# alex-petrenko/sample-factory

Measured on AMD Instinct MI355X. Metric: env-steps/sec (whole node), 4096 envs, 84x84x4 obs, higher is better.
Workload: dtype f32

## Files before the change

### include/sf_hip.h

```cpp
#ifndef SF_HIP_H
#define SF_HIP_H

#include <stdint.h>

#ifdef __cplusplus
extern "C" {
#endif

#define SF_OK 0
#define SF_ERR_ARG (-1)
#define SF_ERR_LAUNCH (-2)
#define SF_ERR_UNSUPPORTED (-3)

const char *sf_last_error(void);
int sf_abi_version(void);

int sf_valid_mask(const int32_t *policy_id, const float *policy_version, uint8_t *valids, uint8_t *valids_flat,
                  float *actions, int num_actions, float *log_prob_actions, int E, int T, int my_policy_id,
                  int train_step, int max_policy_lag, int32_t *num_invalid, void *stream);

int sf_gae_returns(float *rewards, const uint8_t *dones, const uint8_t *time_outs, const float *values,
                   const uint8_t *valids, const double *rms_stats, int E, int T, float gamma, float gae_lambda,
                   int value_bootstrap, float *advantages, float *returns, void *stream);

int sf_moments(const float *x, const uint8_t *valids, const int32_t *index, int64_t offset, int64_t n, int dense_x,
               double *moments, void *stream);
int sf_rms_update(const double *stats_in, const double *moments, double *stats_out, void *stream);
int sf_rms_apply(float *x, int64_t n, const double *stats, int denormalize, void *stream);

int sf_obsnorm_moments(const void *in, int in_u8, int64_t stride, const int32_t *index, int64_t offset, int traj_T,
                       int64_t n, int D, float sub_mean, float inv_scale, double *sum, double *sumsq, void *stream);
int sf_obsnorm_update(double *mean, double *var, const double *count_in, double *count_out, const double *sum,
                      const double *sumsq, int64_t n, int D, float *mu_tab, float *rstd_tab, void *stream);
int sf_obsnorm_apply(const void *in, int in_u8, int64_t stride, const int32_t *index, int64_t offset, int traj_T,
                     int64_t n, int D, int C, int HW, float sub_mean, float inv_scale, const float *mu,
                     const float *rstd, float *out, void *stream);

int sf_rnn_cell_fwd(int kind, const float *gx, const float *gh, const float *h_prev, int64_t ld_h, const float *c_prev,
                    int64_t ld_c, const float *keep, int C, int H, float *gates_out, float *h_out, float *c_out,
                    float *h_next, float *c_next, void *stream);
int sf_rnn_cell_bwd(int kind, const float *dh, const float *dc_in, const float *gates, const float *h_prev,
                    int64_t ld_h, const float *c_prev, int64_t ld_c, const float *c_out, int C, int H, float *dgx,
                    float *dgh, float *dh_direct, float *dc_prev, void *stream);
int sf_rows_add_scale(const float *a, const float *b, const float *keep, int64_t C, int H, float *y, void *stream);

int sf_vtrace(const float *params, int ld_params, const float *values, int ld_values, const float *actions,
              const float *old_logp, const float *rewards, const uint8_t *dones, const int32_t *index, int64_t offset,
              int64_t n, int A, int action_kind, int recurrence, float gamma, float rho_hat, float c_hat, float *vs,
              float *adv, const int32_t *head_n , int num_heads,
              void *stream);

typedef struct {
    float clip_ratio;
    float clip_value;
    float value_loss_coeff;
    float exploration_coeff;
    float kl_coeff;
    int32_t exploration_kind;
    int32_t action_kind;
    int32_t dense_adv;
    int32_t num_heads;
    int32_t head_n[8];
    int32_t old_values_T;
} sf_loss_cfg;

int sf_ppo_loss(const float *params, int ld_params, const float *values, int ld_values, const float *actions,
                const float *old_logp, const float *old_params, const float *old_values, const float *adv,
                const float *targets, const uint8_t *valids, const int32_t *index, int64_t offset, int64_t n, int A,
                const sf_loss_cfg *h_cfg, const double *moments, double *sums, float *g_params, float *g_values,
                float *ratio_out ,
                void *stream);
int sf_loss_scalars(const double *sums, const double *moments, const sf_loss_cfg *h_cfg, float *out, void *stream);
int sf_train_summaries(const uint8_t *valids, const float *ratio, const float *values, int ld_values,
                       const float *old_values, int old_values_T, const float *actions, int num_actions, const float *adv,
                       int dense_adv, const int32_t *policy_id, const float *policy_version, const float *action_logits,
                       int A, const int32_t *index, int64_t offset, int64_t n, int my_policy_id, int train_step,
                       float clip_ratio, const float *exp_avg_sq, int64_t P, double *out, void *stream);

int sf_minibatch_indices(int32_t *out, int64_t experience_size, int recurrence, int shuffle, uint32_t seed,
                         uint32_t epoch, void *stream);
int sf_minibatch_expand(const int32_t *chunk_starts, int32_t *out, int64_t experience_size, int recurrence,
                        void *stream);

int sf_grad_sumsq(const float *g, int64_t P, double *sumsq, void *stream);
int sf_adam_step(float *p, const float *g, float *m, float *v, int64_t P, int step, float lr, float beta1,
                 float beta2, float eps, float max_grad_norm, const double *sumsq, float grad_scale,
                 const uint32_t *skip_flag, void *stream);
int sf_adam_step_dlr(float *p, const float *g, float *m, float *v, int64_t P, int step, const float *lr_dev,
                     float lr_scale, float beta1, float beta2, float eps, float max_grad_norm, const double *sumsq,
                     float grad_scale, const uint32_t *skip_flag, void *stream);
int sf_lr_kl_adaptive(const float *kl, float *lr_dev, float threshold, float lr_min, float lr_max, float *lr_out,
                      void *stream);
int sf_clock_probe(unsigned long long *out, int spin_cycles, void *stream);

int sf_lamb_step(float *p, const float *g, float *m, float *v, float *scratch, const uint8_t *seg_id, double *seg_sums,
                 int64_t P, int num_segments, int step, float lr, float beta1, float beta2, float eps,
                 float weight_decay, float min_trust, float max_grad_norm, const double *sumsq, float grad_scale,
                 const uint32_t *skip_flag, void *stream);

int sf_sample_write_step(const float *logits, int ld_logits, const float *values, int ld_values, int B, int A, int T,
                         int t, uint32_t seed, uint32_t step, uint32_t row0, float policy_version, int deterministic,
                         int action_kind, float *traj_actions,
                         float *traj_logits, float *traj_logp, float *traj_values, float *traj_policy_version,
                         int32_t *env_actions, void *stream);

int sf_sample_write_step_masked(const float *logits, int ld_logits, const float *values, int ld_values,
                                const uint8_t *action_mask, int64_t ld_mask, int B, int A, int T, int t, uint32_t seed,
                                uint32_t step, uint32_t row0, float policy_version, int deterministic,
                                float *traj_actions, float *traj_logits, float *traj_logp, float *traj_values,
                                float *traj_policy_version, int32_t *env_actions, void *stream);

int sf_sample_write_step_tuple(const float *logits, int ld_logits, const float *values, int ld_values, int B,
                               int num_heads, const int32_t *head_n, int T, int t, uint32_t seed, uint32_t step,
                               uint32_t row0, float policy_version, int deterministic, float *traj_actions,
                               float *traj_logits, float *traj_logp, float *traj_values, float *traj_policy_version,
                               int32_t *env_actions, void *stream);

int sf_traj_write_env_step(const float *rewards, const uint8_t *terminated, const uint8_t *truncated, int B, int T,
                           int t, float reward_scale, float reward_clip, int policy_id, float *traj_rewards,
                           uint8_t *traj_dones, uint8_t *traj_time_outs, int32_t *traj_policy_id, float *ep_return,
                           int32_t *ep_len, double *ep_stats, void *stream);

int sf_synth_vec_step(float *state, const float *actions, int64_t act_stride, float *obs_out, int64_t out_stride, int B,
                      int D, int A, int env0, uint32_t seed, uint32_t step, int reset, float *rewards,
                      uint8_t *terminated, void *stream);

int sf_h2d_rows(void *dst, int64_t dst_pitch, const void *src, int64_t src_pitch, int64_t row_bytes, int64_t rows,
                void *stream);
int sf_copy_rows(void *dst, int64_t dst_pitch, const void *src, int64_t src_pitch, int64_t row_bytes, int64_t rows,
                 void *stream);

int sf_synth_obs(uint8_t *obs, int64_t env_stride, int B, int env0, int64_t obs_bytes, uint32_t seed, uint32_t step,
                 void *stream);
int sf_synth_step(const int32_t *actions, int B, int env0, int num_actions, uint32_t seed, uint32_t step,
                  float *rewards, uint8_t *terminated, void *stream);

typedef struct {
    int32_t Cin, H, W;
    int32_t Cout, KH, KW, stride;
    int32_t OH, OW;
    int32_t in_u8;
    int32_t relu;
    int32_t traj_T;
    float sub_mean, inv_scale;
} sf_conv_desc;

int64_t sf_conv_fwd_workspace(int64_t n, const sf_conv_desc *h_desc);
int sf_conv_fwd(const void *in, int64_t in_sample_stride, const int32_t *index, int64_t offset, const float *w,
                const float *bias, float *out, int64_t n, const sf_conv_desc *h_desc, void *workspace,
                int64_t workspace_bytes, void *stream);
int64_t sf_conv_wgrad_workspace(int64_t n, const sf_conv_desc *h_desc);
int sf_conv_wgrad(const void *in, int64_t in_sample_stride, const int32_t *index, int64_t offset, const float *dout,
                  float *dw, float *db, int64_t n, const sf_conv_desc *h_desc, void *workspace, void *stream);
int sf_conv_dgrad(const float *dout, const float *w, const float *in_act, float *din, int64_t n,
                  const sf_conv_desc *h_desc, void *stream);
int sf_conv_relu_mask_supported(int64_t n, const sf_conv_desc *h_desc);
int sf_conv_fwd_relu_mask(const void *in, int64_t in_sample_stride, const int32_t *index, int64_t offset, const float *w,
                          const float *bias, float *out, uint32_t *relu_mask, int64_t n, const sf_conv_desc *h_desc,
                          void *stream);
int sf_conv_wgrad_relu_mask(const void *in, int64_t in_sample_stride, const int32_t *index, int64_t offset,
                            const float *dout, const uint32_t *relu_mask, float *dw, float *db, int64_t n,
                            const sf_conv_desc *h_desc, void *workspace, void *stream);

int sf_conv_norm_supported(int64_t n, const sf_conv_desc *h_desc);
int sf_conv_fwd_norm(const void *in, int64_t in_sample_stride, const int32_t *index, int64_t offset, const float *mu,
                     const float *rstd, const float *w, const float *bias, float *out, int64_t n,
                     const sf_conv_desc *h_desc, void *stream);
int sf_conv_wgrad_norm(const void *in, int64_t in_sample_stride, const int32_t *index, int64_t offset, const float *mu,
                       const float *rstd, const float *dout, float *dw, float *db, int64_t n, const sf_conv_desc *h_desc,
                       void *workspace, void *stream);

int sf_mlp2_fwd(const float *x, int64_t x_stride, int64_t n, int D, float sub_mean, float inv_scale, const float *mu,
                const float *rstd, const float *w1, const float *b1, int H1, const float *w2, const float *b2, int H2,
                int act, float *out, void *stream);

int sf_rnn_store_state(const float *h, const float *c, const uint8_t *dones, int64_t done_stride, float *out,
                       int64_t out_stride, int64_t B, int H, void *stream);

int sf_rnn_chunk_setup(const uint8_t *dones, const uint8_t *valids, const float *rnn_states, const int32_t *index,
                       int64_t offset, int Cn, int R, int S, int traj_T, float *keep_tm, float *h0, void *stream);

int sf_lstm_seq_supported(int Cn, int H);
int sf_lstm_seq_fwd(const float *gx, const float *whh, const float *bhh, const float *keep, float *gates, float *hprev,
                    float *hout, float *cprev, float *cout, uint32_t *sync, int R, int Cn, int H, int env_major,
                    void *stream);
int sf_lstm_seq_bwd(const float *dout, const float *gates, const float *cprev, const float *cout, const float *keep,
                    const float *whh, float *dgx, uint32_t *sync, int R, int Cn, int H, int env_major, void *stream);

int sf_gru_seq_fwd(const float *gx, const float *whh, const float *bhh, const float *keep, float *gates, float *hprev,
                   float *hout, uint32_t *sync, int R, int Cn, int H, int env_major, void *stream);
int sf_gru_seq_bwd(const float *dout, const float *gates, const float *hprev, const float *keep, const float *whh,
                   float *dgx, float *dgh, uint32_t *sync, int R, int Cn, int H, int env_major, void *stream);

int sf_seq_fwd_x_supported(int Cn, int H, int Kx);
int sf_lstm_seq_fwd_x(const float *x, const float *wih_t, const float *bih, int Kx, const float *whh, const float *bhh,
                      const float *keep, float *gates, float *hprev, float *hout, float *cprev, float *cout,
                      uint32_t *sync, int R, int Cn, int H, int env_major, void *stream);
int sf_gru_seq_fwd_x(const float *x, const float *wih_t, const float *bih, int Kx, const float *whh, const float *bhh,
                     const float *keep, float *gates, float *hprev, float *hout, uint32_t *sync, int R, int Cn, int H,
                     int env_major, void *stream);

#define SF_DP_UNIQUE_ID_BYTES 128
int sf_dp_unique_id(void *out_id);
int sf_dp_comm_create(const void *id_bytes, int nranks, int rank, void **comm_out);
int sf_dp_comm_destroy(void *comm);
int sf_dp_comm_info(void *comm, int *nranks, int *rank);
int sf_allreduce_grads(void *comm, float *grads, int64_t n, void *stream);
int sf_dp_allreduce_f64(void *comm, double *buf, int64_t n, int op, void *stream);
int sf_dp_broadcast(void *comm, void *buf, int64_t nbytes, int root, void *stream);

#define SF_DP_IPC_HANDLE_BYTES 64
int sf_dp_oneshot_create(int nranks, int rank, int64_t max_bytes, void **ctx_out, void *handle_out);
int sf_dp_oneshot_connect(void *ctx, const void *all_handles );
int sf_dp_oneshot_allreduce_f32(void *ctx, float *buf, int64_t n, void *stream);
int sf_dp_oneshot_allreduce_f64(void *ctx, double *buf, int64_t n, int op, void *stream);
int sf_dp_oneshot_status(void *ctx);
int sf_dp_oneshot_destroy(void *ctx);

int sf_tanh_scale_fwd(float *x, int ld, int64_t n, int col0, int ncols, float scale, void *stream);
int sf_tanh_scale_bwd(float *g, const float *y, int ld, int64_t n, int col0, int ncols, float scale, void *stream);

int sf_linear_fwd_dual_supported(int64_t n, int N, int K1, int K2);
int sf_linear_fwd_dual(const float *a1, int64_t lda1, const float *w1t, const float *bias1, int K1, const float *a2,
                       int64_t lda2, const float *w2t, const float *bias2, int K2, float *out, int64_t n, int N,
                       int gru_H, void *stream);

int sf_conv_fwd_t_supported(int64_t n, const sf_conv_desc *desc);
int64_t sf_conv_fwd_t_workspace(int64_t n, const sf_conv_desc *desc);
int sf_conv_fwd_t(const float *in, int64_t in_sample_stride, const float *wt, const float *bias, float *out,
                  int64_t n, const sf_conv_desc *desc, void *workspace, int64_t workspace_bytes, void *stream);
int sf_transpose(const float *w, float *wt, int K, int N, void *stream);

int sf_conv_kernel_name(int op, int64_t n, const sf_conv_desc *desc, int split_k_allowed, char *out, int cap);
int sf_linear_fwd(const float *in, const float *w, const float *bias, float *out, int64_t M, int K, int N, int relu,
                  void *stream);
int64_t sf_linear_wgrad_workspace(int64_t M, int K, int N);
// ... 31 lines not shown
```

### sample_factory_amd/algo/learning/learner.py

```python
from __future__ import annotations

import glob
import time
import os
from os.path import join
from typing import Dict, List, Optional, Tuple

import numpy as np
import torch

from sample_factory_amd import lib
from sample_factory_amd.algo.learning.dp import ReplicaGroup
from sample_factory_amd.algo.utils.tensor_dict import TensorDict
from sample_factory_amd.envs.spaces import (action_head_sizes, calc_num_action_parameters, calc_num_actions, is_box,
                                             is_discrete)
from sample_factory_amd.model.actor_critic import ActorCritic
from sample_factory_amd.model.model_factory import create_actor_critic
from sample_factory_amd.utils.attr_dict import AttrDict
from sample_factory_amd.utils.decay import LinearDecay

LEARNER_ENV_STEPS, POLICY_ID_KEY, STATS_KEY, TRAIN_STATS = "learner_env_steps", "policy_id", "stats", "train"


class LearningRateScheduler:
# ... 75 lines not shown
    def __init__(self, policy_id, policy_versions: torch.Tensor, serial_mode: bool = True):
        self.policy_id = policy_id
        self.actor_critic = None
        self.policy_versions = policy_versions
        self.device = None
        self.policy_lock = _NullLock()

    def init(self, actor_critic, policy_version, device):
        self.actor_critic, self.device = actor_critic, device
        self.policy_versions[self.policy_id] = policy_version


class Learner:
    def __init__(self, cfg, env_info, policy_versions_tensor: torch.Tensor, policy_id: int, param_server,
                 process_group=None):
        self.cfg = cfg
        self.env_info = env_info
        self.policy_id = policy_id
        self.policy_versions_tensor = policy_versions_tensor
        self.param_server = param_server
        self.device: Optional[torch.device] = None
        self.actor_critic: Optional[ActorCritic] = None
        self.curr_lr: Optional[float] = None
        self.lr_scheduler: Optional[LearningRateScheduler] = None
        self.train_step = 0
        self.env_steps = 0
        self.best_performance = -1e9
        self.new_cfg: Optional[Dict] = None
        self.policy_to_load = None
        self.is_initialized = False
        self.last_summary: Dict = {}
        self.pg = process_group
        dp_on = process_group is not None or (getattr(cfg, "data_parallel", False) and torch.distributed.is_initialized())
        self.group = ReplicaGroup(process_group, bool(getattr(cfg, "dp_force_collectives", False)),
                                  bool(getattr(cfg, "dp_native_rccl", False)),
                                  oneshot_bytes=int(getattr(cfg, "dp_oneshot_bytes", 0) or 0)) if dp_on else None
        self.world = self.group.world if self.group is not None else 1
        self.dp = self.group is not None and self.group.on
        self._grad_norms: List[float] = []

    def _all_reduce(self, t: torch.Tensor) -> None:
        if self.dp:
            self.group.all_reduce_sum(t)

    def init(self):
        cfg = self.cfg
        if cfg.exploration_loss not in ("entropy", "symmetric_kl"):
            raise NotImplementedError(f"{cfg.exploration_loss} not supported!")
        if cfg.optimizer not in ("adam", "lamb"):
            raise RuntimeError(f"Unknown optimizer {cfg.optimizer}")
        if cfg.seed is not None:
            torch.manual_seed(cfg.seed)
            np.random.seed(cfg.seed)
        if not torch.cuda.is_available():
            raise lib.SfHipError("Learner.init(): no GPU visible. sample_factory_amd has no CPU path.")
        lib.load()
        self.device = torch.device("cuda", torch.cuda.current_device())
        ar = self._all_reduce if self.dp else None
        cfg.dp_world = self.world
        self.actor_critic = create_actor_critic(cfg, self.env_info.obs_space, self.env_info.action_space, self.device,
                                                all_reduce=ar)
        self.actor_critic.train()
        if self.dp:
            self.group.broadcast(self.actor_critic.flat_params, src=0)
            self.actor_critic.params_changed()
        P = self.actor_critic.num_flat
        self.exp_avg = torch.zeros(P, dtype=torch.float32, device=self.device)
        self.exp_avg_sq = torch.zeros(P, dtype=torch.float32, device=self.device)
        self.adam_step_count = 0
        self._dp_reduce_each_mb = True
        self._dp_split = None
        ac_ = self.actor_critic
        if self.dp and getattr(cfg, "dp_overlap", True) and hasattr(ac_, "_segs") and ac_.rnn_kind is None:
            sizes = [L.K * L.N for L in ac_.layers]
            li = int(np.argmax(sizes))
            if li > 0 and sum(sizes[li:]) * 2 >= sum(sizes):
                self._dp_split = li
        self._lamb = None
        dev = self.device
        self._num_invalid = torch.zeros(1, dtype=torch.int32, device=dev)
        self._moments = torch.zeros(3, dtype=torch.float64, device=dev)
        self._sums = torch.zeros(8, dtype=torch.float64, device=dev)
        self._sumsq = torch.zeros(1, dtype=torch.float64, device=dev)
        self._scalars = None
        A = calc_num_action_parameters(self.env_info.action_space)
        self.num_action_params = A
        self.num_actions = calc_num_actions(self.env_info.action_space)
        self._refresh_loss_cfg()
        self.load_from_checkpoint(self.policy_id)
        self.param_server.init(self.actor_critic, self.train_step, self.device)
        self.policy_versions_tensor[self.policy_id] = self.train_step
        self.lr_scheduler = get_lr_scheduler(cfg)
        self.curr_lr = cfg.learning_rate if self.curr_lr is None else self.curr_lr
        self.is_initialized = True
        state_dict = None if cfg.serial_mode else self.actor_critic.state_dict()
        return self.policy_id, state_dict, self.device, self.train_step

    @staticmethod
    def checkpoint_dir(cfg, policy_id):
        d = join(experiment_dir(cfg), f"checkpoint_p{policy_id}")
        os.makedirs(d, exist_ok=True)
        return d

    @staticmethod
    def get_checkpoints(checkpoints_dir, pattern="checkpoint_*"):
        return sorted(glob.glob(join(checkpoints_dir, pattern)))

    @staticmethod
    def load_checkpoint(checkpoints, device):
        if not checkpoints:
            return None
        return torch.load(checkpoints[-1], map_location="cpu", weights_only=False)

    def _get_checkpoint_dict(self):
        ac = self.actor_critic
        names = [n for n, _ in ac.ref_param_shapes()]
        m, v = ac.flat_to_ref(self.exp_avg), ac.flat_to_ref(self.exp_avg_sq)
        opt_state = {i: dict(step=torch.tensor(float(self.adam_step_count)), exp_avg=m[n], exp_avg_sq=v[n])
                     for i, n in enumerate(names)} if self.adam_step_count > 0 else {}
        opt = dict(state=opt_state, param_groups=[dict(
            lr=self.curr_lr, betas=(self.cfg.adam_beta1, self.cfg.adam_beta2), eps=self.cfg.adam_eps, weight_decay=0,
            amsgrad=False, maximize=False, foreach=None, capturable=False, differentiable=False, fused=None,
            decoupled_weight_decay=False, params=list(range(len(names))))])
        return dict(train_step=self.train_step, env_steps=self.env_steps, best_performance=self.best_performance,
                    model=ac.state_dict(), optimizer=opt, curr_lr=self.curr_lr)

    def _save_impl(self, name_prefix: str, name_suffix: str, keep_checkpoints: int) -> bool:
        if not self.is_initialized:
            return False
        d = self.checkpoint_dir(self.cfg, self.policy_id)
        tmp = join(d, f"{name_prefix}_temp")
        name = join(d, f"{name_prefix}_{self.train_step:09d}_{self.env_steps}{name_suffix}.pth")
        torch.save(self._get_checkpoint_dict(), tmp)
        os.rename(tmp, name)
        while len(cps := self.get_checkpoints(d, f"{name_prefix}_*")) > keep_checkpoints:
            if os.path.isfile(cps[0]):
                os.remove(cps[0])
        return True

    def save(self) -> bool:
        return self._save_impl("checkpoint", "", self.cfg.keep_checkpoints)

    def save_milestone(self) -> None:
        d = join(self.checkpoint_dir(self.cfg, self.policy_id), "milestones")
        os.makedirs(d, exist_ok=True)
        torch.save(self._get_checkpoint_dict(), join(d, f"checkpoint_{self.train_step:09d}_{self.env_steps}.pth"))

    def save_best(self, policy_id, metric, metric_value) -> bool:
        if policy_id != self.policy_id:
            return False
        p = 3
        if metric_value - self.best_performance > 1 / 10 ** p:
            self.best_performance = metric_value
            return self._save_impl("best", f"_{metric}_{metric_value:.{p}f}", 1)
        return False

    def _load_state(self, cp, load_progress=True):
        if load_progress:
            self.train_step, self.env_steps = cp["train_step"], cp["env_steps"]
            self.best_performance = cp.get("best_performance", self.best_performance)
        ac = self.actor_critic
        ac.load_state_dict(cp["model"])
        st = cp["optimizer"].get("state", {})
        if st:
            names = [n for n, _ in ac.ref_param_shapes()]
            m = {n: st[i]["exp_avg"] for i, n in enumerate(names)}
# ... 76 lines not shown
        heads = ac.forward_heads(last, E, sample_stride=0 if multi else obs.stride(0), tag="boot", rnn=rnn)[-1]
        lib.copy_rows(batch["values"][:, T], heads[:, 0])
        adv = torch.empty((E, T), dtype=torch.float32, device=self.device)
        ret = torch.empty((E, T), dtype=torch.float32, device=self.device)
        buff = AttrDict()
        if not cfg.with_vtrace:
            rms = ac.returns_normalizer.stats if cfg.normalize_returns else None
            lib.gae_returns(batch["rewards"], batch["dones"], batch["time_outs"], batch["values"], batch["valids"],
                            rms, cfg.gamma, cfg.gae_lambda, cfg.value_bootstrap, adv, ret)
            buff.advantages, buff.returns = adv.view(N), ret.view(N)
        elif cfg.value_bootstrap:
            lib.gae_returns(batch["rewards"], batch["dones"], batch["time_outs"], batch["values"], batch["valids"],
                            None, cfg.gamma, cfg.gae_lambda, True, adv, ret)
        buff.obs = obs
        buff.actions = batch["actions"].view(N, self.num_actions)
        buff.action_logits = batch["action_logits"].view(N, self.num_action_params)
        buff.log_prob_actions = batch["log_prob_actions"].view(N)
        buff.rewards = batch["rewards"].view(N)
        buff.dones = batch["dones"].view(N)
        buff.policy_id, buff.policy_version = batch["policy_id"].view(N), batch["policy_version"].view(N)
        if cfg.use_rnn:
            buff.rnn_states = batch["rnn_states"]
        buff["values"] = batch["values"]
        buff.valids = valids_flat
        buff.E, buff.T = E, T
        if cfg.normalize_returns and not cfg.with_vtrace:
            ac.returns_normalizer(buff.returns)
        num_invalids = int(self._num_invalid.item())
        if self.dp:
            t = torch.tensor([num_invalids], dtype=torch.int64, device=self.device)
            self._all_reduce(t)
            self._global_invalids = int(t.item())
        else:
            self._global_invalids = num_invalids
        return buff, N, num_invalids

    def _get_minibatches(self, batch_size, experience_size):
        cfg = self.cfg
        assert cfg.rollout % cfg.recurrence == 0
        assert experience_size % batch_size == 0, f"experience size: {experience_size}, batch size: {batch_size}"
        n_mb = cfg.num_batches_per_epoch
        if n_mb == 1:
            return [(None, 0, experience_size)]
        assert n_mb * batch_size == experience_size, \
            f"dataset of {experience_size} samples != num_batches_per_epoch {n_mb} x batch_size {batch_size}"
        if cfg.shuffle_minibatches:
            idx = torch.empty(experience_size, dtype=torch.int32, device=self.device)
            if getattr(cfg, "device_shuffle", False):
                seed = (cfg.seed or 0) * 7919 + self.policy_id
                lib.minibatch_indices(idx, experience_size, cfg.recurrence, True, seed, self._shuffle_epoch)
                self._shuffle_epoch += 1
            else:
                starts = np.random.permutation(np.arange(0, experience_size, cfg.recurrence))
                starts_dev = torch.from_numpy(starts.astype(np.int32)).to(self.device, non_blocking=True)
                lib.minibatch_expand(starts_dev, idx, experience_size, cfg.recurrence)
            return [(idx[i * batch_size:(i + 1) * batch_size], 0, batch_size) for i in range(experience_size // batch_size)]
        return [(None, i * batch_size, batch_size) for i in range(n_mb)]

    _shuffle_epoch = 0

    def _calculate_losses(self, mb: AttrDict, num_invalids: int):
        from sample_factory_amd.algo.utils.action_distributions import get_action_distribution
        buff, part = (mb if isinstance(mb, tuple) else (mb, None))
        if part is None:
            part = (None, 0, buff.E * buff.T)
        acts, g_heads, sc = self._losses_native(buff, part, num_invalids)
        index, offset, n = part
        heads = acts[-1]
        A = self.num_action_params
        space = self.env_info.action_space
        dist = get_action_distribution(space, heads[:n, 1:1 + A])
        dist.raw_logits, dist.values = heads[:n, 1:1 + A], heads[:n, 0]
        rows = index.long() if index is not None else torch.arange(offset, offset + n, device=self.device)
        kl_old = dist.kl_divergence(get_action_distribution(space, buff.action_logits[rows]))[buff.valids[rows]]
        summaries = AttrDict(adv_mean=sc[6], adv_std=sc[7], num_valid=sc[8], entropy=sc[9], kl_divergence_max=sc[5],
                             kl_old_mean=sc[4].clone(), ratio=self._ratio[:n], values=heads[:n, 0], g_heads=g_heads)
        return dist, sc[0].clone(), sc[1].clone(), kl_old, sc[2].clone(), sc[3].clone(), summaries

    def _losses_native(self, buff: AttrDict, mb, num_invalids: int, scalars_out: Optional[torch.Tensor] = None,
                       moments: Optional[torch.Tensor] = None):
        cfg, ac = self.cfg, self.actor_critic
        index, offset, n = mb
        A = self.num_action_params
        rnn = None
        if cfg.use_rnn:
            R, Cn = cfg.recurrence, n // cfg.recurrence
            keep_tm = ac._buf(("rnn", "keep_tm"), (R, Cn))
            h0 = ac._buf(("rnn", "h0"), (Cn, buff.rnn_states.shape[-1]))
            lib.rnn_chunk_setup(buff.dones, buff.valids, buff.rnn_states, index, offset, Cn, R, keep_tm, h0, traj_T=buff.T)
            rnn = dict(R=R, h0=h0, keep_tm=keep_tm)
        acts = ac.forward_heads(buff.obs, n, sample_stride=ac.obs_elems, index=index, offset=offset,
                                traj_T=buff.T, tag="train", rnn=rnn)
        heads = acts[-1]
        ld = ac.heads_ld
        params, values = heads[:, 1:], heads[:, 0]
        g_heads = ac._zbuf(("g", "heads"), (n, ld))
        if cfg.with_vtrace:
            vs = ac._buf(("vt", "vs"), (n,))
            adv = ac._buf(("vt", "adv"), (n,))
            lib.vtrace(params, ld, values, ld, buff.actions, buff.log_prob_actions, buff.rewards, buff.dones, index,
                       offset, n, A, self.loss_cfg.action_kind, cfg.recurrence, cfg.gamma, cfg.vtrace_rho,
                       cfg.vtrace_c, vs, adv, head_sizes=self._head_sizes)
            lib.moments(adv, buff.valids, index, n, self._moments, offset=offset, dense_x=True)
            adv_arr, tgt_arr = adv, vs
        elif moments is None:
            lib.moments(buff.advantages, buff.valids, index, n, self._moments, offset=offset)
            adv_arr, tgt_arr = buff.advantages, buff.returns
        else:
            adv_arr, tgt_arr = buff.advantages, buff.returns
        if moments is None:
            moments = self._moments
            self._all_reduce(moments)
        self._ratio = ac._buf(("loss", "ratio"), (n,))
        self.loss_cfg.old_values_T = buff.T
        lib.ppo_loss(params, ld, values, ld, buff.actions, buff.log_prob_actions, buff.action_logits, buff["values"],
                     adv_arr, tgt_arr, buff.valids, index, offset, n, A, self.loss_cfg, moments, self._sums,
                     g_heads[:, 1:], g_heads[:, 0], ratio_out=self._ratio)
        self._last_mb = (index, offset, n, values, adv_arr)
        if self.dp and self._dp_reduce_each_mb:
            self.group.loss_sums(self._sums)
        out = scalars_out if scalars_out is not None else torch.zeros(16, dtype=torch.float32, device=self.device)
        lib.loss_scalars(self._sums, moments, self.loss_cfg, out)
        return acts, g_heads, out

    def _epoch_moments(self, buff: AttrDict, minibatches) -> Optional[torch.Tensor]:
        if not self.dp or self.cfg.with_vtrace or not getattr(self.cfg, "dp_epoch_moments", True):
            return None
        tab = self.actor_critic._buf(("loss", "epoch_moments"), (len(minibatches), 3), dtype=torch.float64)
        for i, (index, offset, n) in enumerate(minibatches):
            lib.moments(buff.advantages, buff.valids, index, n, tab[i], offset=offset)
        self._all_reduce(tab)
        return tab

    def _train(self, buff: AttrDict, batch_size: int, experience_size: int, num_invalids: int) -> Optional[AttrDict]:
        cfg, ac = self.cfg, self.actor_critic
        early_stopping_tolerance = 1e-6
        prev_epoch_actor_loss = 1e9
        recent_kls: List[float] = []
        num_sgd_steps = 0
        n_mb = cfg.num_batches_per_epoch
        self._scalars = ac._buf(("loss", "scalars"), (cfg.num_epochs * n_mb, 16))
        global_size = experience_size * self.world
        need_kl_each_mb = self.lr_scheduler.invoke_after_each_minibatch() and isinstance(self.lr_scheduler, KlAdaptiveScheduler)
        self._dp_reduce_each_mb = need_kl_each_mb
        lr_on_device = need_kl_each_mb and cfg.optimizer == "adam"
        if lr_on_device:
            if not hasattr(self, "_lr_dev"):
                self._lr_dev = torch.zeros(1, dtype=torch.float32, device=self.device)
            self._lr_dev.fill_(float(self.curr_lr))
        self._grad_norms = []
        skip = ac.rnn_abort_word() if hasattr(ac, "rnn_abort_word") else None
        if skip is not None:
            ac.rnn_abort_clear()
        for epoch in range(cfg.num_epochs):
            minibatches = self._get_minibatches(batch_size, experience_size)
            mom_tab = self._epoch_moments(buff, minibatches)
            for batch_num, mb in enumerate(minibatches):
                row = self._scalars[epoch * n_mb + batch_num]
                acts, g_heads, _ = self._losses_native(buff, mb, num_invalids, row,
                                                       moments=None if mom_tab is None else mom_tab[batch_num])
                index, offset, n = mb
                if self._dp_split is not None:
                    cut = ac._segs[self._dp_split][0]
                    pending = []
                    ac.backward(acts, g_heads, buff.obs, n, sample_stride=ac.obs_elems, index=index, offset=offset,
                                traj_T=buff.T,
                                on_layer_done=lambda li: pending.append(self.group.all_reduce_grads_async(
                                    ac.flat_grads[cut:])) if li == self._dp_split else None)
                    self.group.all_reduce_grads(ac.flat_grads[:cut])
                    for work in pending:
                        work.wait()
                else:
                    ac.backward(acts, g_heads, buff.obs, n, sample_stride=ac.obs_elems, index=index, offset=offset,
                                traj_T=buff.T)
                    if self.dp:
                        self.group.all_reduce_grads(ac.flat_grads)
                actual_lr = self.curr_lr
                valid_frac = 1.0
                if self._global_invalids > 0:
                    valid_frac = (global_size - self._global_invalids) / global_size
                    actual_lr = self.curr_lr * valid_frac
                self.adam_step_count += 1
                use_clip = cfg.max_grad_norm > 0.0
                if use_clip or getattr(cfg, "record_grad_norm", False):
                    lib.grad_sumsq(ac.flat_grads, self._sumsq)
                    if getattr(cfg, "record_grad_norm", False):
                        self._grad_norms.append(float(self._sumsq.sqrt().item()))
                if cfg.optimizer == "lamb":
                    if self._lamb is None:
                        seg, nseg = ac.tensor_segment_ids()
                        self._lamb = (seg, nseg, torch.empty_like(ac.flat_params),
                                      torch.zeros(128, dtype=torch.float64, device=self.device))
                    seg, nseg, scratch, seg_sums = self._lamb
                    lib.lamb_step(ac.flat_params, ac.flat_grads, self.exp_avg, self.exp_avg_sq, scratch, seg, seg_sums,
                                  nseg, self.adam_step_count, actual_lr, cfg.adam_beta1, cfg.adam_beta2, cfg.adam_eps,
                                  1e-4, 0.01, cfg.max_grad_norm if use_clip else 0.0, self._sumsq if use_clip else None,
                                  skip_flag=skip)
                elif lr_on_device:
                    lib.adam_step_dlr(ac.flat_params, ac.flat_grads, self.exp_avg, self.exp_avg_sq, self.adam_step_count,
                                      self._lr_dev, valid_frac, cfg.adam_beta1, cfg.adam_beta2, cfg.adam_eps,
                                      cfg.max_grad_norm if use_clip else 0.0, self._sumsq if use_clip else None,
                                      skip_flag=skip)
                else:
                    lib.adam_step(ac.flat_params, ac.flat_grads, self.exp_avg, self.exp_avg_sq, self.adam_step_count,
                                  actual_lr, cfg.adam_beta1, cfg.adam_beta2, cfg.adam_eps,
                                  cfg.max_grad_norm if use_clip else 0.0, self._sumsq if use_clip else None,
                                  skip_flag=skip)
                ac.params_changed()
                num_sgd_steps += 1
                self.train_step += 1
                if lr_on_device:
                    sch = self.lr_scheduler
                    lib.lr_kl_adaptive(row[4:5], self._lr_dev, sch.threshold, sch.min_lr, sch.max_lr, lr_out=row[10:11])
                elif need_kl_each_mb:
                    recent_kls.append(float(row[4].item()))
                    self.curr_lr = self.lr_scheduler.update(self.curr_lr, recent_kls)
                elif self.lr_scheduler.invoke_after_each_minibatch():
                    self.curr_lr = self.lr_scheduler.update(self.curr_lr, recent_kls)
                self.policy_versions_tensor[self.policy_id] = self.train_step
            blk = self._scalars[epoch * n_mb:(epoch + 1) * n_mb]
            if self.dp and not need_kl_each_mb:
                flag = (skip.to(torch.float32) if skip is not None else blk.new_zeros(1)).expand(blk.shape[0], 1)
                pack = torch.cat([blk[:, [0, 1, 2, 3, 4, 9, 5]], flag], dim=1).contiguous()
                self.group.reduce_sum_max(pack, (6, 7))
                blk[:, [0, 1, 2, 3, 4, 9, 5]] = pack[:, :7]
                aborted = skip is not None and bool(pack[0, 7].item() != 0)
            elif self.dp and skip is not None:
                aborted = bool(self.group.all_reduce_max(skip.to(torch.float32)).item() != 0)
            else:
                aborted = skip is not None and ac.rnn_pass_aborted()
            rows = blk.cpu()
            if aborted:
                raise lib.SfHipError(
                    "a fused recurrent sequence pass was aborted (a work-group never arrived: is the GPU shared with "
                    "another process?); the optimiser steps after it were skipped, the weights are those of the last "
                    "good SGD step; set SF_LSTM_SEQ=0 to use the per-step kernels")
            actor_losses = (rows[:, 0] + rows[:, 1] + rows[:, 2]).double().numpy()
            if lr_on_device:
                self.curr_lr = float(rows[-1, 10])
                actual_lr = self.curr_lr * valid_frac
            if not need_kl_each_mb or lr_on_device:
                recent_kls.extend(rows[:, 4].double().tolist())
            if self.lr_scheduler.invoke_after_each_epoch():
                self.curr_lr = self.lr_scheduler.update(self.curr_lr, recent_kls)
            new_epoch_actor_loss = float(np.mean(actor_losses))
            if abs(prev_epoch_actor_loss - new_epoch_actor_loss) < early_stopping_tolerance:
                break
            prev_epoch_actor_loss = new_epoch_actor_loss
        last = rows[-1]
        stats = AttrDict(lr=self.curr_lr, actual_lr=actual_lr, env_steps=self.env_steps,
                         policy_loss=float(last[0]), exploration_loss=float(last[1]),
                         kl_loss=float(last[2]), value_loss=float(last[3]), kl_divergence=float(last[4]),
                         kl_divergence_max=float(last[5]), adv_mean=float(last[6]), adv_std=float(last[7]),
                         entropy=float(last[9]), loss=float(last[0] + last[1] + last[2] + last[3]),
                         num_sgd_steps=num_sgd_steps)
        if self._should_save_summaries():
            stats.update(self._record_summaries(buff))
            self._last_summary_time = time.time()
        self.last_summary = stats
        return stats

    _last_summary_time = 0.0
    _summary_rate_decay = LinearDecay([(0, 2.0), (100000, 60.0), (1000000, 120.0)])

    def _should_save_summaries(self) -> bool:
        every = self._summary_rate_decay.at(float(self.train_step))
        return time.time() - self._last_summary_time >= every or getattr(self.cfg, "summaries_every_train", False)

    def _record_summaries(self, buff: AttrDict) -> Dict[str, float]:
        index, offset, n, values, adv_arr = self._last_mb
        if not hasattr(self, "_summ"):
            self._summ = torch.empty(24, dtype=torch.float64, device=self.device)
        ld = values.stride(0) if values.dim() == 1 else 1
        lib.train_summaries(buff.valids, self._ratio, values, ld, buff["values"], buff.T, buff.actions, self.num_actions,
                            adv_arr, bool(self.cfg.with_vtrace), buff.policy_id, buff.policy_version, buff.action_logits,
                            self.num_action_params, index, offset, n, self.policy_id, self.train_step,
                            self.loss_cfg.clip_ratio, self.exp_avg_sq, self._summ)
        o = self._summ.cpu().tolist()
        rows, nv, ns = o[0], o[1], o[2]
        has_v, has_s = nv > 0, ns > 0
        return dict(
            valids_fraction=nv / rows, same_policy_fraction=ns / rows, value=o[3] / rows,
            ratio_mean=o[4] / nv if has_v else 0.0, ratio_min=o[8] if has_v else 1.0, ratio_max=o[9] if has_v else 1.0,
            fraction_clipped=o[5] / nv if has_v else 0.0, value_delta=o[6] / rows, value_delta_max=o[10],
            act_min=o[11], act_max=o[12], adv_min=o[13], adv_max=o[14], max_abs_logprob=o[15],
            version_diff_avg=o[7] / ns if has_s else 0.0, version_diff_min=o[16] if has_s else 0.0,
            version_diff_max=o[17] if has_s else 0.0, grad_norm=float(self._sumsq.sqrt().item()),
            adam_max_second_moment=o[18])

    def train(self, batch: TensorDict) -> Optional[Dict]:
        self._maybe_update_cfg()
# ... 12 lines not shown
```

### sample_factory_amd/csrc/sf_nn.hip

```cpp
#include "sf_common.h"
#include <stdlib.h>
#ifndef SF_GLDS_ABLATE
#define SF_GLDS_ABLATE 0
#endif
#include <type_traits>

#define STREAM(s) reinterpret_cast<hipStream_t>(s)

typedef float f32x16 __attribute__((ext_vector_type(16)));

struct FastDiv {
    uint32_t d, mul, shr;
};
static inline FastDiv make_fastdiv(uint32_t d) {
    FastDiv f;
    f.d = d;
    if (d <= 1) { f.mul = 0; f.shr = 0; return f; }
    uint32_t s = 0;
    while ((1u << s) < d) ++s;
    f.mul = (uint32_t)((((uint64_t)1) << (31 + s)) / d + 1);
    f.shr = s - 1;
    return f;
}
__host__ __device__ __forceinline__ uint32_t fdiv(uint32_t n, const FastDiv &f) {
// ... 505 lines not shown
                    ra[s] = load_act_raw<MODE_GENERIC>(g, in, base, po, (uint32_t)(k0row + kg[s]), aok[s]);
            }
        }
#pragma unroll
        for (int s = 0; s < T::SB; ++s) {
            const int64_t m = mc + bkk0 + s * BROWS;
            bok[s] = m < mend;
            rb[s] = load_row_raw<VECB>(dy, bok[s] ? m : mbeg, n0 + bcg, N);
        }
    };
    const bool do_colsum = partial_b != nullptr && blockIdx.x == 0 && tid < BN;
    float colacc = 0.f;
    if (mbeg < mend) gload(mbeg);
    for (int64_t mc = mbeg; mc < mend; mc += 32) {
        __syncthreads();
#pragma unroll
        for (int s = 0; s < T::SA; ++s) {
            const int lrow = FR ? (tid & 31) : (tid >> 5) + 8 * s;
            *reinterpret_cast<float4 *>(&As[lrow * LDA + kg[s]]) =
                act_finish<MODE>(g, ra[s], MODE != MODE_GENERIC || aok[s]);
        }
        const bool tail = mc + 32 > mend;
#pragma unroll
        for (int s = 0; s < T::SB; ++s)
            *reinterpret_cast<float4 *>(&Bs[(bkk0 + s * BROWS) * LDB + bcg]) =
                (VECB && !tail) ? rb[s] : row_finish(rb[s], bok[s], n0 + bcg, N);
        __syncthreads();
        if (mc + 32 < mend) gload(mc + 32);
        if (do_colsum) {
#pragma unroll 8
            for (int kk = 0; kk < 32; ++kk) colacc += Bs[kk * LDB + tid];
        }
        mma_chunk<T::TM, T::TN, LDA, LDB>(As, Bs, wm * T::TM * 32, wn * T::TN * 32, lane, acc);
    }
    if (do_colsum && n0 + tid < N) partial_b[(int64_t)blockIdx.z * N + n0 + tid] = colacc;
    float *dst = partial + (int64_t)blockIdx.z * K * N;
#pragma unroll
    for (int tm = 0; tm < T::TM; ++tm)
#pragma unroll
        for (int tn = 0; tn < T::TN; ++tn) {
            const int n = n0 + wn * T::TN * 32 + tn * 32 + (lane & 31);
#pragma unroll
            for (int r = 0; r < 16; ++r) {
                const int k = k0row + wm * T::TM * 32 + tm * 32 + FRAG_ROW(r, lane);
                if (k < K && n < N) dst[(int64_t)k * N + n] = acc[tm][tn][r];
            }
        }
}

__global__ __launch_bounds__(256) void k_reduce_partials(const float *__restrict__ partial, float *__restrict__ out,
                                                         int64_t n, int Z) {
    for (int64_t i = (int64_t)blockIdx.x * blockDim.x + threadIdx.x; i < n; i += (int64_t)gridDim.x * blockDim.x) {
        float s[8] = {0.f, 0.f, 0.f, 0.f, 0.f, 0.f, 0.f, 0.f};
        int z = 0;
        for (; z + 8 <= Z; z += 8) {
#pragma unroll
            for (int j = 0; j < 8; ++j) s[j] += partial[(int64_t)(z + j) * n + i];
        }
        for (int j = 0; z < Z; ++z, ++j) s[j] += partial[(int64_t)z * n + i];
        out[i] = ((s[0] + s[1]) + (s[2] + s[3])) + ((s[4] + s[5]) + (s[6] + s[7]));
    }
}

__global__ __launch_bounds__(256) void k_reduce_partials_tree(const float *__restrict__ partial, float *__restrict__ out,
                                                              int64_t n, int Z) {
    __shared__ float sm[8][33];
    const int li = threadIdx.x & 31, zg = threadIdx.x >> 5;
    const int64_t i = (int64_t)blockIdx.x * 32 + li;
    const int zper = (Z + 7) / 8, z0 = zg * zper, z1 = z0 + zper < Z ? z0 + zper : Z;
    float s[8] = {0.f, 0.f, 0.f, 0.f, 0.f, 0.f, 0.f, 0.f};
    if (i < n) {
        int z = z0;
        for (; z + 8 <= z1; z += 8) {
#pragma unroll
            for (int j = 0; j < 8; ++j) s[j] += partial[(int64_t)(z + j) * n + i];
        }
        for (int j = 0; z < z1; ++z, ++j) s[j] += partial[(int64_t)z * n + i];
    }
    sm[zg][li] = ((s[0] + s[1]) + (s[2] + s[3])) + ((s[4] + s[5]) + (s[6] + s[7]));
    __syncthreads();
    if (zg == 0 && i < n)
        out[i] = ((sm[0][li] + sm[1][li]) + (sm[2][li] + sm[3][li])) + ((sm[4][li] + sm[5][li]) + (sm[6][li] + sm[7][li]));
}
static void launch_reduce_partials(const float *partial, float *out, int64_t n, int Z, hipStream_t st) {
    static const int tree_on = getenv("SF_REDUCE_TREE") ? atoi(getenv("SF_REDUCE_TREE")) : 1;
    if (tree_on && Z >= 64 && (n + 255) / 256 < 256)
        k_reduce_partials_tree<<<dim3((unsigned)((n + 31) / 32)), dim3(256), 0, st>>>(partial, out, n, Z);
    else
        k_reduce_partials<<<dim3((unsigned)((n + 255) / 256 < 2048 ? (n + 255) / 256 : 2048)), dim3(256), 0, st>>>(partial, out, n, Z);
}

template <int BM, int BN, int WM, int WN, bool VEC>
__global__ __launch_bounds__(256) void k_conv_dgrad(ConvG g, const float *__restrict__ dy,
                                                    const float *__restrict__ w, const float *__restrict__ in_act,
                                                    float *__restrict__ din, int64_t nsamples) {
    using T = Tile<BM, BN, WM, WN>;
    constexpr int LDA = BM + 1, LDB = BN + 1;
    __shared__ __attribute__((aligned(16))) float As[32 * LDA];
    __shared__ __attribute__((aligned(16))) float Bs[32 * LDB];
    const int tid = threadIdx.x, lane = tid & 63, wave = tid >> 6;
    const int wm = wave / WN, wn = wave % WN;
    const int ph = blockIdx.z / g.S, pw = blockIdx.z % g.S;
    const int Hc = (g.H - ph + g.S - 1) / g.S, Wc = (g.W - pw + g.S - 1) / g.S;
    const int KHs = (g.KH - ph + g.S - 1) / g.S, KWs = (g.KW - pw + g.S - 1) / g.S;
    const int64_t Mc = nsamples * Hc * Wc;
    const int64_t m0 = (int64_t)blockIdx.x * BM;
    if (m0 >= Mc || Hc <= 0 || Wc <= 0) return;
    const int n0 = blockIdx.y * BN;
    const int Cin = g.Cin, Cout = g.Cout;
    const int Kp = KHs * KWs * Cout;

    const int kq = (tid & 7) * 4;
    const FastDiv fHW = g.dHcWc[blockIdx.z], fW = g.dWc[blockIdx.z], fKWs = g.dKWs[blockIdx.z];
    int arow[T::SA], aih[T::SA], aiw[T::SA];
    bool aval[T::SA];
    const uint32_t HcWc = (uint32_t)(Hc * Wc);
#pragma unroll
    for (int s = 0; s < T::SA; ++s) {
        const int64_t m = m0 + (tid >> 3) + 32 * s;
        aval[s] = m < Mc;
        const uint32_t mm = aval[s] ? (uint32_t)m : 0u;
        const uint32_t smp = fdiv(mm, fHW), pix = mm - smp * HcWc;
        aih[s] = (int)fdiv(pix, fW);
        aiw[s] = (int)pix - aih[s] * Wc;
        arow[s] = (int)(smp * (uint32_t)(g.OH * g.OW)) + aih[s] * g.OW + aiw[s];
    }
    const bool kfull = (Kp & 31) == 0;
    f32x16 acc[T::TM][T::TN];
    ZERO_ACC(acc);

    float4 ra[T::SA], rb[T::SB];
    bool aok[T::SA], bok = true;
    int ncol = 0;
    auto gload = [&](int k0) {
        const int k = k0 + kq;
        const bool kval = k < Kp;
        const int kc = kval ? k : 0;
        const int tap = (int)fdiv((uint32_t)kc, g.dCout);
        const int n = kc - tap * Cout;
        ncol = n;
        const int a = (int)fdiv((uint32_t)tap, fKWs), b = tap - a * KWs;
        const int drow = a * g.OW + b;
#pragma unroll
        for (int s = 0; s < T::SA; ++s) {
            const int oh = aih[s] - a, ow = aiw[s] - b;
            aok[s] = kval && aval[s] && oh >= 0 && oh < g.OH && ow >= 0 && ow < g.OW;
            const int row = aok[s] ? arow[s] - drow : 0;
            ra[s] = load_row_raw<VEC>(dy, row, n, Cout);
        }
        const int wrow = ((ph + a * g.S) * g.KW + (pw + b * g.S)) * Cin;
        bok = kval;
#pragma unroll
        for (int s = 0; s < T::SB; ++s) {
            const int c = n0 + (tid >> 3) + 32 * s;
            rb[s] = load_row_raw<VEC>(w, wrow + (c < Cin ? c : 0), n, Cout);
        }
    };
    if (Kp > 0) gload(0);
    for (int k0 = 0; k0 < Kp; k0 += 32) {
        __syncthreads();
#pragma unroll
        for (int s = 0; s < T::SA; ++s) {
            const float4 v = row_finish(ra[s], aok[s], ncol, Cout);
            As[(kq + 0) * LDA + (tid >> 3) + 32 * s] = v.x;
            As[(kq + 1) * LDA + (tid >> 3) + 32 * s] = v.y;
            As[(kq + 2) * LDA + (tid >> 3) + 32 * s] = v.z;
            As[(kq + 3) * LDA + (tid >> 3) + 32 * s] = v.w;
        }
#pragma unroll
        for (int s = 0; s < T::SB; ++s) {
            const float4 v = (VEC && kfull) ? rb[s] : row_finish(rb[s], bok, ncol, Cout);
            Bs[(kq + 0) * LDB + (tid >> 3) + 32 * s] = v.x;
// ... 1073 lines not shown
```

### sample_factory_amd/csrc/sf_rl.hip

```cpp
#include "sf_common.h"

thread_local char sf_err_buf[512] = "";

extern "C" const char *sf_last_error(void) { return sf_err_buf; }
extern "C" int sf_abi_version(void) { return 19; }

#define STREAM(s) reinterpret_cast<hipStream_t>(s)

__device__ __forceinline__ float clampf(float x, float lo, float hi) { return fminf(fmaxf(x, lo), hi); }

__global__ __launch_bounds__(256) void k_valid_mask(const int32_t *__restrict__ policy_id,
                                                    const float *__restrict__ policy_version,
                                                    uint8_t *__restrict__ valids, uint8_t *__restrict__ valids_flat,
                                                    float *__restrict__ actions,
                                                    int num_actions, float *__restrict__ logp, int E, int T,
                                                    int my_pid, int train_step, int max_lag,
                                                    int32_t *__restrict__ num_invalid) {
    const int64_t i = (int64_t)blockIdx.x * blockDim.x + threadIdx.x;
    const int64_t N = (int64_t)E * T;
    const bool in = i < N;
    bool valid = true;
    if (in) {
        const int64_t e = i / T;
        const int t = (int)(i - e * T);
// ... 99 lines not shown
    }
    float cum = 0.0f;
    for (int t0 = ((T - 1) / GAE_TC) * GAE_TC; t0 >= 0; t0 -= GAE_TC) {
        const int tc = min(GAE_TC, T - t0);
        const GaeTile fr = gae_fetch_f32(rewards, T, e0, E, t0, tc, tid);
        const GaeTile fd = gae_fetch_u8(dones, T, e0, E, t0, tc, tid);
        const GaeTile fv = gae_fetch_f32(values, T + 1, e0, E, t0, tc + 1, tid);
        const GaeTile fa = gae_fetch_u8(valids, T + 1, e0, E, t0, tc + 1, tid);
        GaeTile ft;
        if (value_bootstrap) ft = gae_fetch_u8(time_outs, T, e0, E, t0, tc, tid);
        __syncthreads();
        gae_put(s_r, fr, tc, tid);
        gae_put(s_d, fd, tc, tid);
        gae_put(s_v, fv, tc + 1, tid);
        gae_put(s_va, fa, tc + 1, tid);
        if (value_bootstrap) gae_put(s_to, ft, tc, tid);
        __syncthreads();
        if (tid < 64) {
            for (int c = tc; c >= 0; --c) {
                float v = s_v[lane][c];
                if (denorm) v = clampf(v, -5.0f, 5.0f) * sigma + mu;
                s_v[lane][c] = v;
            }
            for (int c = tc - 1; c >= 0; --c) {
                const float v = s_v[lane][c], vn = s_v[lane][c + 1];
                const float valid = s_va[lane][c], valid_n = s_va[lane][c + 1];
                const float done = s_d[lane][c];
                float r = s_r[lane][c];
                if (value_bootstrap) {
                    r = r + ((gamma * v) * s_to[lane][c]) * done;
                    s_r[lane][c] = r;
                }
                const float a = (r - v) * valid;
                const float b = (1.0f - done) * ((gamma * vn) * valid_n);
                const float delta = a + b;
                const float disc = gl * valid + (1.0f - valid);
                cum = delta + (disc * cum) * (1.0f - done);
                s_adv[lane][c] = cum;
                s_ret[lane][c] = cum + valid * v;
            }
        }
        __syncthreads();
        gae_tile_store_f32(s_adv, adv_out, T, e0, E, t0, tc, tid);
        gae_tile_store_f32(s_ret, ret_out, T, e0, E, t0, tc, tid);
        if (value_bootstrap) gae_tile_store_f32(s_r, rewards, T, e0, E, t0, tc, tid);
    }
}

extern "C" int sf_gae_returns(float *rewards, const uint8_t *dones, const uint8_t *time_outs, const float *values,
                              const uint8_t *valids, const double *rms_stats, int E, int T, float gamma,
                              float gae_lambda, int value_bootstrap, float *advantages, float *returns,
                              void *stream) {
    SF_REQUIRE(E > 0 && T > 0, "sf_gae_returns: bad shape E=%d T=%d", E, T);
    SF_REQUIRE(rewards && dones && values && valids && advantages && returns, "sf_gae_returns: null pointer");
    SF_REQUIRE(!value_bootstrap || time_outs, "sf_gae_returns: value_bootstrap needs time_outs");
    const float gl = (float)((double)gamma * (double)gae_lambda);
    k_gae_returns<<<dim3((unsigned)((E + 63) / 64)), dim3(GAE_NT), 0, STREAM(stream)>>>(
        rewards, dones, time_outs, values, valids, rms_stats, E, T, gamma, gl, value_bootstrap, advantages, returns);
    return sf_launch_status("sf_gae_returns");
}

__global__ __launch_bounds__(256) void k_moments(const float *__restrict__ x, const uint8_t *__restrict__ valids,
                                                 const int32_t *__restrict__ index, int64_t offset, int64_t n,
                                                 int dense_x, double *__restrict__ moments) {
    __shared__ double lds[4 * 3];
    double acc[3] = {0.0, 0.0, 0.0};
    for (int64_t i = (int64_t)blockIdx.x * blockDim.x + threadIdx.x; i < n; i += (int64_t)gridDim.x * blockDim.x) {
        const int64_t j = index ? (int64_t)index[i] : offset + i;
        if (!valids || valids[j]) {
            const double v = (double)x[dense_x ? i : j];
            acc[0] += v;
            acc[1] += v * v;
            acc[2] += 1.0;
        }
    }
    sf_block_sum<3>(acc, lds);
    if (threadIdx.x == 0) {
        atomicAdd(&moments[0], acc[0]);
        atomicAdd(&moments[1], acc[1]);
        atomicAdd(&moments[2], acc[2]);
    }
}

extern "C" int sf_moments(const float *x, const uint8_t *valids, const int32_t *index, int64_t offset, int64_t n,
                          int dense_x, double *moments, void *stream) {
    SF_REQUIRE(x && moments && n >= 0 && offset >= 0, "sf_moments: bad args");
    int rc = sf_hip_status(hipMemsetAsync(moments, 0, 3 * sizeof(double), STREAM(stream)), "sf_moments memset");
    if (rc || n == 0) return rc;
    const int64_t blocks = (n + 255) / 256;
    k_moments<<<dim3((unsigned)(blocks < 2048 ? blocks : 2048)), dim3(256), 0, STREAM(stream)>>>(
        x, valids, index, offset, n, dense_x, moments);
    return sf_launch_status("sf_moments");
}

__global__ void k_rms_update(const double *__restrict__ stats_in, const double *__restrict__ moments,
                             double *__restrict__ stats_out) {
    if (threadIdx.x != 0 || blockIdx.x != 0) return;
    const double n = moments[2];
    const double mean = stats_in[0], var = stats_in[1], count = stats_in[2];
    if (n <= 0.0) { stats_out[0] = mean; stats_out[1] = var; stats_out[2] = count; return; }
    const double bm64 = moments[0] / n;
    const double bv64 = (moments[1] - moments[0] * bm64) / (n - 1.0);
    const double batch_mean = (double)(float)bm64, batch_var = (double)(float)bv64;
    const double delta = batch_mean - mean;
    const double tot = count + n;
    const double new_mean = mean + delta * n / tot;
    const double M2 = var * count + batch_var * n + (delta * delta) * count * n / tot;
    stats_out[0] = new_mean;
    stats_out[1] = M2 / tot;
    stats_out[2] = tot;
}

extern "C" int sf_rms_update(const double *stats_in, const double *moments, double *stats_out, void *stream) {
    SF_REQUIRE(stats_in && moments && stats_out, "sf_rms_update: null pointer");
    k_rms_update<<<dim3(1), dim3(64), 0, STREAM(stream)>>>(stats_in, moments, stats_out);
    return sf_launch_status("sf_rms_update");
}

__global__ __launch_bounds__(256) void k_rms_apply(float *__restrict__ x, int64_t n,
                                                   const double *__restrict__ stats, int denormalize) {
    const float mu = (float)stats[0];
    const float sigma = sqrtf((float)stats[1] + 1e-5f);
    const float inv = 1.0f / sigma;
    for (int64_t i = (int64_t)blockIdx.x * blockDim.x + threadIdx.x; i < n; i += (int64_t)gridDim.x * blockDim.x) {
        float v = x[i];
        if (denormalize) v = clampf(v, -5.0f, 5.0f) * sigma + mu;
        else v = clampf((v - mu) * inv, -5.0f, 5.0f);
        x[i] = v;
    }
}

extern "C" int sf_rms_apply(float *x, int64_t n, const double *stats, int denormalize, void *stream) {
    SF_REQUIRE(x && stats && n >= 0, "sf_rms_apply: bad args");
    if (n == 0) return SF_OK;
    const int64_t blocks = (n + 255) / 256;
    k_rms_apply<<<dim3((unsigned)(blocks < 2048 ? blocks : 2048)), dim3(256), 0, STREAM(stream)>>>(x, n, stats,
                                                                                                   denormalize);
    return sf_launch_status("sf_rms_apply");
}

template <int MAXA>
__device__ __forceinline__ float action_logp(const float *__restrict__ z, int A, int action_kind,
                                             const float *__restrict__ act_row) {
    if (action_kind == 0) {
        float zz[MAXA];
        float mx = -INFINITY;
#pragma unroll
        for (int k = 0; k < MAXA; ++k) { zz[k] = k < A ? z[k] : -INFINITY; mx = fmaxf(mx, zz[k]); }
        float se = 0.f;
#pragma unroll
        for (int k = 0; k < MAXA; ++k) if (k < A) se += expf(zz[k] - mx);
        const float lse = logf(se);
        const int a = (int)act_row[0];
        float r = 0.f;
#pragma unroll
        for (int k = 0; k < MAXA; ++k) if (k == a) r = (zz[k] - mx) - lse;
        return r;
    } else {
        const int D = A / 2;
        float r = 0.f;
        for (int k = 0; k < D; ++k) {
            const float mu = z[k], sd = clampf(expf(z[D + k]), 1e-4f, 1e4f);
            const float a = act_row[k];
            r += -((a - mu) * (a - mu)) / (2.f * (sd * sd)) - logf(sd) - 0.91893853320467274178f;
        }
        return r;
    }
}

struct HeadsDev {
    int num_heads, head_n[8];
};
__device__ __host__ __forceinline__ int heads_action_cols(const int *head_n, int num_heads) {
    int c = 0;
    for (int h = 0; h < num_heads; ++h) c += head_n[h] > 0 ? 1 : -head_n[h];
// ... 446 lines not shown
                    off += nh;
                }
                const bool in_v = (v - vo) >= -h.clip_value && (v - vo) <= h.clip_value;
                float dvl;
                if (l1 > l2) dvl = 2.f * (v - R);
                else if (l2 > l1) dvl = in_v ? 2.f * (vclip - R) : 0.f;
                else dvl = (v - R) + (in_v ? (vclip - R) : 0.f);
                g_values[i * ldv] = h.value_coeff * inv_n * dvl;
            } else {
                for (int k = 0; k < A; ++k) gz[k] = 0.f;
                g_values[i * ldv] = 0.f;
            }
        }
    }
    const int lane = threadIdx.x & 63, wave = threadIdx.x >> 6;
    kl_max = sf_wave_max(kl_max);
    if (lane == 0) lds_max[wave] = kl_max;
    sf_block_sum<4>(acc, lds);
    if (threadIdx.x == 0) {
        if (sym_pass) { atomicAdd(&sums[7], acc[0]); return; }
        atomicAdd(&sums[0], acc[0]);
        atomicAdd(&sums[1], acc[1]);
        atomicAdd(&sums[2], acc[2]);
        atomicAdd(&sums[3], acc[3]);
        const float m = fmaxf(fmaxf(lds_max[0], lds_max[1]), fmaxf(lds_max[2], lds_max[3]));
        if (m > -1.0f) atomic_max_float(&sums[4], m);
    }
}

template <int MAXA>
__global__ __launch_bounds__(256) void k_symkl_sum(const float *__restrict__ params, int ldp,
                                                   const uint8_t *__restrict__ valids,
                                                   const int32_t *__restrict__ index, int64_t offset, int64_t n, int A,
                                                   double *__restrict__ out) {
    __shared__ double lds[4];
    const int64_t i = (int64_t)blockIdx.x * blockDim.x + threadIdx.x;
    double acc[1] = {0.0};
    if (i < n) {
        const int64_t d = index ? (int64_t)index[i] : offset + i;
        if (valids[d]) {
            const float *z = params + i * ldp;
            float zz[MAXA];
            float mx = -INFINITY;
#pragma unroll
            for (int k = 0; k < MAXA; ++k) { zz[k] = k < A ? z[k] : -INFINITY; mx = fmaxf(mx, zz[k]); }
            float se = 0.f;
#pragma unroll
            for (int k = 0; k < MAXA; ++k) if (k < A) se += expf(zz[k] - mx);
            const float lse = logf(se), u = 1.0f / (float)A, lu = logf(u);
            float a1 = 0.f, a2 = 0.f;
#pragma unroll
            for (int k = 0; k < MAXA; ++k)
                if (k < A) { const float lp = (zz[k] - mx) - lse; a1 += expf(lp) * (lp - lu); a2 += u * (lu - lp); }
            acc[0] = 0.5f * (a1 + a2);
        }
    }
    sf_block_sum<1>(acc, lds);
    if (threadIdx.x == 0) atomicAdd(out, acc[0]);
}

__global__ void k_symkl_gate(double *__restrict__ sums, const double *__restrict__ moments) {
    if (threadIdx.x || blockIdx.x) return;
    const float m = (float)(sums[7] / moments[2]);
    sums[6] = (isfinite(m) && m <= 30.0f) ? 1.0 : 0.0;
}

static LossDev make_loss_dev(const sf_loss_cfg *c) {
    LossDev h;
    h.clip_hi = (float)(1.0 + (double)c->clip_ratio);
    h.clip_lo = (float)(1.0 / (1.0 + (double)c->clip_ratio));
    h.clip_value = c->clip_value;
    h.value_coeff = c->value_loss_coeff;
    h.expl_coeff = c->exploration_coeff;
    h.kl_coeff = c->kl_coeff;
    h.expl_kind = c->exploration_coeff == 0.f ? 0 : c->exploration_kind;
    h.action_kind = c->action_kind;
    h.dense_adv = c->dense_adv;
    h.num_heads = c->num_heads > 1 ? c->num_heads : 1;
    for (int i = 0; i < 8; ++i) h.head_n[i] = c->num_heads > 1 ? c->head_n[i] : 0;
    h.ov_T = c->old_values_T > 0 ? c->old_values_T : 0;
    return h;
}

extern "C" int sf_ppo_loss(const float *params, int ld_params, const float *values, int ld_values,
                           const float *actions, const float *old_logp, const float *old_params,
                           const float *old_values, const float *adv, const float *targets, const uint8_t *valids,
                           const int32_t *index, int64_t offset, int64_t n, int A, const sf_loss_cfg *h_cfg,
                           const double *moments, double *sums, float *g_params, float *g_values, float *ratio_out,
                           void *stream) {
    SF_REQUIRE(ld_params >= A && ld_values >= 1, "sf_ppo_loss: bad strides");
    SF_REQUIRE(params && values && actions && old_logp && old_params && old_values && adv && targets && valids &&
                   h_cfg && moments && sums && g_params && g_values,
               "sf_ppo_loss: null pointer");
    SF_REQUIRE(n > 0 && A > 0 && A <= 128, "sf_ppo_loss: bad shape n=%lld A=%d", (long long)n, A);
    SF_REQUIRE(h_cfg->action_kind == 0 || (h_cfg->action_kind == 1 && A % 2 == 0), "sf_ppo_loss: bad action_kind");
    SF_REQUIRE(!(h_cfg->exploration_kind == 2 && h_cfg->action_kind != 0 && h_cfg->exploration_coeff != 0.f),
               "sf_ppo_loss: symmetric_kl exploration loss needs a categorical distribution");
    const LossDev h = make_loss_dev(h_cfg);
    int rc = sf_hip_status(hipMemsetAsync(sums, 0, 8 * sizeof(double), STREAM(stream)), "sf_ppo_loss memset");
    if (rc) return rc;
    const dim3 grid((unsigned)((n + 255) / 256)), block(256);
#define PL_DISPATCH(KERNEL, ...)                                                        \
    do {                                                                                \
        if (A <= 8) KERNEL<8><<<grid, block, 0, STREAM(stream)>>>(__VA_ARGS__);         \
        else if (A <= 32) KERNEL<32><<<grid, block, 0, STREAM(stream)>>>(__VA_ARGS__);  \
        else KERNEL<128><<<grid, block, 0, STREAM(stream)>>>(__VA_ARGS__);              \
    } while (0)
    if (h.action_kind == 0 && h.num_heads > 1) {
        int tot = 0;
        SF_REQUIRE(h.num_heads <= 8, "sf_ppo_loss: at most 8 action heads");
        bool any_box = false;
        for (int i = 0; i < h.num_heads; ++i) {
            SF_REQUIRE(h.head_n[i] != 0, "sf_ppo_loss: empty action head");
            tot += h.head_n[i] > 0 ? h.head_n[i] : -2 * h.head_n[i];
            any_box = any_box || h.head_n[i] < 0;
        }
        SF_REQUIRE(tot == A, "sf_ppo_loss: head sizes sum to %d, A = %d", tot, A);
        SF_REQUIRE(!(any_box && h.expl_kind == 2),
                   "sf_ppo_loss: symmetric_kl exploration loss needs categorical heads only (the reference's "
                   "ContinuousActionDistribution has no symmetric_kl_with_uniform_prior)");
        if (h.expl_kind == 2) {
            k_ppo_loss_md<<<grid, block, 0, STREAM(stream)>>>(params, ld_params, values, ld_values, actions, old_logp, old_params,
                                                              old_values, adv, targets, valids, index, offset, n, A, h, moments,
                                                              sums, g_params, g_values, nullptr, 1);
            k_symkl_gate<<<dim3(1), dim3(64), 0, STREAM(stream)>>>(sums, moments);
        }
        k_ppo_loss_md<<<grid, block, 0, STREAM(stream)>>>(params, ld_params, values, ld_values, actions, old_logp, old_params,
                                                          old_values, adv, targets, valids, index, offset, n, A, h, moments, sums,
                                                          g_params, g_values, ratio_out, 0);
        return sf_launch_status("sf_ppo_loss");
    }
    if (h.expl_kind == 2) {
        PL_DISPATCH(k_symkl_sum, params, ld_params, valids, index, offset, n, A, sums + 7);
        k_symkl_gate<<<dim3(1), dim3(64), 0, STREAM(stream)>>>(sums, moments);
    }
    PL_DISPATCH(k_ppo_loss, params, ld_params, values, ld_values, actions, old_logp, old_params, old_values, adv, targets, valids, index,
                offset, n, A, h, moments, sums, g_params, g_values, ratio_out);
#undef PL_DISPATCH
    return sf_launch_status("sf_ppo_loss");
}

__global__ void k_loss_scalars(const double *__restrict__ sums, const double *__restrict__ moments, LossDev h,
                               float *__restrict__ out) {
    if (threadIdx.x || blockIdx.x) return;
    const double n = moments[2];
    const double mean64 = moments[0] / n;
    const double var64 = (moments[1] - moments[0] * mean64) / (n - 1.0);
    out[0] = (float)(-(sums[0] / n));
    if (h.expl_kind == 1) out[1] = (float)(-(double)h.expl_coeff * (sums[1] / n));
    else if (h.expl_kind == 2) {
        float m = (float)(sums[1] / n);
        if (!isfinite(m)) m = 0.f;
        out[1] = h.expl_coeff * fminf(m, 30.0f);
    } else out[1] = 0.f;
    out[2] = (float)((double)h.kl_coeff * (sums[2] / n));
    out[3] = (float)((double)h.value_coeff * (sums[3] / n));
    out[4] = (float)(sums[2] / n);
    out[5] = (float)sums[4];
    out[6] = (float)mean64;
    out[7] = (float)sqrt(var64 > 0.0 ? var64 : 0.0);
    out[8] = (float)n;
    out[9] = (float)(sums[1] / n);
}

extern "C" int sf_loss_scalars(const double *sums, const double *moments, const sf_loss_cfg *h_cfg, float *out,
                               void *stream) {
    SF_REQUIRE(sums && moments && h_cfg && out, "sf_loss_scalars: null pointer");
    k_loss_scalars<<<dim3(1), dim3(64), 0, STREAM(stream)>>>(sums, moments, make_loss_dev(h_cfg), out);
    return sf_launch_status("sf_loss_scalars");
}

constexpr int SUMM_NS = 8, SUMM_NM = 11, SUMM_OUT = 24;
struct SummArgs {
    const uint8_t *valids;
    const float *ratio, *values, *old_values, *actions, *adv, *policy_version, *action_logits;
    const int32_t *policy_id, *index;
    int64_t offset, n;
    int ld_values, old_values_T, num_actions, A, dense_adv, my_pid;
    float train_step, clip_lo, clip_hi;
};
__device__ __forceinline__ void atomic_minmax_d(double *addr, double v, bool is_max) {
    unsigned long long *a = reinterpret_cast<unsigned long long *>(addr);
    unsigned long long old = *a, assumed;
    do {
        assumed = old;
        const double cur = __longlong_as_double((long long)assumed);
        if (is_max ? cur >= v : cur <= v) break;
        old = atomicCAS(a, assumed, (unsigned long long)__double_as_longlong(v));
    } while (assumed != old);
}
__global__ void k_summ_init(double *out) {
    const int i = threadIdx.x;
    if (i >= SUMM_OUT) return;
    const bool is_min = i == 8 || i == 11 || i == 13 || i == 16;
    const bool is_max = i == 9 || i == 10 || i == 12 || i == 14 || i == 15 || i == 17 || i == 18;
    out[i] = is_min ? (double)INFINITY : is_max ? -(double)INFINITY : 0.0;
}
__global__ __launch_bounds__(256) void k_train_summaries(SummArgs p, double *__restrict__ out) {
    __shared__ double lds[4 * SUMM_NS];
    __shared__ float ldm[4 * SUMM_NM];
    double s[SUMM_NS] = {0, 0, 0, 0, 0, 0, 0, 0};
    float mn[4] = {INFINITY, INFINITY, INFINITY, INFINITY};
    float mx[7] = {-INFINITY, -INFINITY, -INFINITY, -INFINITY, -INFINITY, -INFINITY, -INFINITY};
    for (int64_t i = (int64_t)blockIdx.x * blockDim.x + threadIdx.x; i < p.n; i += (int64_t)gridDim.x * blockDim.x) {
        const int64_t d = p.index ? (int64_t)p.index[i] : p.offset + i;
        const bool valid = p.valids[d] != 0, same = p.policy_id[d] == p.my_pid;
        const float v = p.values[i * p.ld_values];
        const int64_t dv_row = p.old_values_T > 0 ? d + d / p.old_values_T : d;
        const float dv = fabsf(v - p.old_values[dv_row]);
        s[0] += 1.0;
        s[1] += valid ? 1.0 : 0.0;
        s[2] += same ? 1.0 : 0.0;
        s[3] += (double)v;
        s[6] += (double)dv;
        mx[1] = fmaxf(mx[1], dv);
        if (valid) {
            const float r = p.ratio[i];
            s[4] += (double)fabsf(1.0f - r);
            s[5] += (r < p.clip_lo ? 1.0 : 0.0) + (r > p.clip_hi ? 1.0 : 0.0);
            mn[0] = fminf(mn[0], r);
            mx[0] = fmaxf(mx[0], r);
        }
        for (int a = 0; a < p.num_actions; ++a) {
            const float x = p.actions[d * p.num_actions + a];
            mn[1] = fminf(mn[1], x);
            mx[2] = fmaxf(mx[2], x);
        }
        const float ad = p.adv[p.dense_adv ? i : d];
        mn[2] = fminf(mn[2], ad);
        mx[3] = fmaxf(mx[3], ad);
        for (int a = 0; a < p.A; ++a) mx[4] = fmaxf(mx[4], fabsf(p.action_logits[d * p.A + a]));
        if (same) {
            const float vd = p.train_step - p.policy_version[d];
            s[7] += (double)vd;
            mn[3] = fminf(mn[3], vd);
            mx[5] = fmaxf(mx[5], vd);
        }
    }
    const int lane = threadIdx.x & 63, wave = threadIdx.x >> 6;
#pragma unroll
    for (int k = 0; k < SUMM_NS; ++k) s[k] = sf_wave_sum(s[k]);
#pragma unroll
    for (int k = 0; k < 4; ++k)
#pragma unroll
        for (int off = 32; off > 0; off >>= 1) mn[k] = fminf(mn[k], __shfl_down(mn[k], off, 64));
#pragma unroll
    for (int k = 0; k < 7; ++k) mx[k] = sf_wave_max(mx[k]);
    if (lane == 0) {
#pragma unroll
        for (int k = 0; k < SUMM_NS; ++k) lds[wave * SUMM_NS + k] = s[k];
#pragma unroll
        for (int k = 0; k < 4; ++k) ldm[wave * SUMM_NM + k] = mn[k];
// ... 187 lines not shown
    SF_REQUIRE(((uintptr_t)g & 15) == 0, "sf_grad_sumsq: gradient buffer must be 16-byte aligned");
    int rc = sf_hip_status(hipMemsetAsync(sumsq, 0, sizeof(double), STREAM(stream)), "sf_grad_sumsq memset");
    if (rc) return rc;
    const int64_t blocks = (P / 4 + 255) / 256;
    k_grad_sumsq<<<dim3((unsigned)(blocks < 1024 ? (blocks ? blocks : 1) : 1024)), dim3(256), 0, STREAM(stream)>>>(
        g, P, sumsq);
    return sf_launch_status("sf_grad_sumsq");
}

struct AdamC {
    float lr_step, bc2_sqrt, w1, b2, w2, eps, max_norm, grad_scale;
};

__device__ __forceinline__ void adam1(float &p, float g, float &m, float &v, const AdamC &c, float coef) {
    g = g * coef;
    m = m + (g - m) * c.w1;
    v = v * c.b2 + (g * g) * c.w2;
    const float denom = sqrtf(v) / c.bc2_sqrt + c.eps;
    p = p - c.lr_step * (m / denom);
}

__global__ __launch_bounds__(256) void k_adam(float *__restrict__ p, const float *__restrict__ g,
                                              float *__restrict__ m, float *__restrict__ v, int64_t P, AdamC c,
                                              const double *__restrict__ sumsq, const uint32_t *__restrict__ skip,
                                              const float *__restrict__ lr_dev) {
    if (skip && *skip) return;
    if (lr_dev) c.lr_step *= *lr_dev;
    float coef = c.grad_scale;
    if (sumsq && c.max_norm > 0.f) {
        const float total = (float)sqrt(*sumsq) * fabsf(c.grad_scale);
        const float cc = c.max_norm / (total + 1e-6f);
        coef = c.grad_scale * fminf(cc, 1.0f);
    }
    const int64_t nvec = P / 4;
    const int64_t tid = (int64_t)blockIdx.x * blockDim.x + threadIdx.x, nt = (int64_t)gridDim.x * blockDim.x;
    float4 *p4 = reinterpret_cast<float4 *>(p), *m4 = reinterpret_cast<float4 *>(m), *v4 = reinterpret_cast<float4 *>(v);
    const float4 *g4 = reinterpret_cast<const float4 *>(g);
    for (int64_t i = tid; i < nvec; i += nt) {
        float4 pp = p4[i], mm = m4[i], vv = v4[i];
        const float4 gg = g4[i];
        adam1(pp.x, gg.x, mm.x, vv.x, c, coef);
        adam1(pp.y, gg.y, mm.y, vv.y, c, coef);
        adam1(pp.z, gg.z, mm.z, vv.z, c, coef);
        adam1(pp.w, gg.w, mm.w, vv.w, c, coef);
        p4[i] = pp; m4[i] = mm; v4[i] = vv;
    }
    for (int64_t i = nvec * 4 + tid; i < P; i += nt) adam1(p[i], g[i], m[i], v[i], c, coef);
}

static int adam_step_impl(float *p, const float *g, float *m, float *v, int64_t P, int step, float lr, float beta1,
                          float beta2, float eps, float max_grad_norm, const double *sumsq, float grad_scale,
                          const uint32_t *skip_flag, const float *lr_dev, void *stream, const char *who) {
    SF_REQUIRE(p && g && m && v && P > 0 && step >= 1, "%s: bad args", who);
    SF_REQUIRE((((uintptr_t)p | (uintptr_t)g | (uintptr_t)m | (uintptr_t)v) & 15) == 0,
               "%s: buffers must be 16-byte aligned", who);
    AdamC c;
    const double bc1 = 1.0 - pow((double)beta1, (double)step), bc2 = 1.0 - pow((double)beta2, (double)step);
    c.lr_step = (float)((double)lr / bc1);
    c.bc2_sqrt = (float)sqrt(bc2);
    c.w1 = (float)(1.0 - (double)beta1);
    c.b2 = beta2;
    c.w2 = (float)(1.0 - (double)beta2);
    c.eps = eps;
    c.max_norm = max_grad_norm;
    c.grad_scale = grad_scale;
    const int64_t blocks = (P / 4 + 255) / 256;
    k_adam<<<dim3((unsigned)(blocks < 2048 ? (blocks ? blocks : 1) : 2048)), dim3(256), 0, STREAM(stream)>>>(
        p, g, m, v, P, c, sumsq, skip_flag, lr_dev);
    return sf_launch_status(who);
}

extern "C" int sf_adam_step(float *p, const float *g, float *m, float *v, int64_t P, int step, float lr, float beta1,
                            float beta2, float eps, float max_grad_norm, const double *sumsq, float grad_scale,
                            const uint32_t *skip_flag, void *stream) {
    return adam_step_impl(p, g, m, v, P, step, lr, beta1, beta2, eps, max_grad_norm, sumsq, grad_scale, skip_flag, nullptr,
                          stream, "sf_adam_step");
}
extern "C" int sf_adam_step_dlr(float *p, const float *g, float *m, float *v, int64_t P, int step, const float *lr_dev,
                                float lr_scale, float beta1, float beta2, float eps, float max_grad_norm,
                                const double *sumsq, float grad_scale, const uint32_t *skip_flag, void *stream) {
    SF_REQUIRE(lr_dev, "sf_adam_step_dlr: null lr_dev");
    return adam_step_impl(p, g, m, v, P, step, lr_scale, beta1, beta2, eps, max_grad_norm, sumsq, grad_scale, skip_flag,
                          lr_dev, stream, "sf_adam_step_dlr");
}

__global__ void k_clock_probe(unsigned long long *__restrict__ out, int spin_cycles) {
    if (threadIdx.x || blockIdx.x) return;
    const unsigned long long w0 = wall_clock64(), c0 = clock64();
    unsigned long long c1 = c0;
    while ((long long)(c1 - c0) < (long long)spin_cycles) c1 = clock64();
    const unsigned long long w1 = wall_clock64();
    out[0] = c1 - c0;
    out[1] = w1 - w0;
}
extern "C" int sf_clock_probe(unsigned long long *out, int spin_cycles, void *stream) {
    SF_REQUIRE(out && spin_cycles > 0, "sf_clock_probe: bad args");
    k_clock_probe<<<dim3(1), dim3(64), 0, STREAM(stream)>>>(out, spin_cycles);
    return sf_launch_status("sf_clock_probe");
}

__global__ void k_lr_kl_adaptive(const float *__restrict__ kl, float *__restrict__ lr_dev, float threshold, float lr_min,
                                 float lr_max, float *__restrict__ lr_out) {
    if (threadIdx.x || blockIdx.x) return;
    const double k = (double)*kl;
    double lr = (double)*lr_dev;
    if (k > 2.0 * (double)threshold) lr = fmax(lr / 1.5, (double)lr_min);
    if (k < 0.5 * (double)threshold) lr = fmin(lr * 1.5, (double)lr_max);
    *lr_dev = (float)lr;
    if (lr_out) *lr_out = (float)lr;
}
extern "C" int sf_lr_kl_adaptive(const float *kl, float *lr_dev, float threshold, float lr_min, float lr_max,
                                 float *lr_out, void *stream) {
    SF_REQUIRE(kl && lr_dev, "sf_lr_kl_adaptive: null pointer");
    k_lr_kl_adaptive<<<dim3(1), dim3(64), 0, STREAM(stream)>>>(kl, lr_dev, threshold, lr_min, lr_max, lr_out);
    return sf_launch_status("sf_lr_kl_adaptive");
}

struct LambC {
    float inv_bc1, inv_bc2_sqrt, w1, b1, b2, w2, eps, wd, max_norm, grad_scale, lr, min_trust;
};
constexpr int LAMB_MAX_SEG = 64;

__global__ __launch_bounds__(256) void k_lamb_dir(const float *__restrict__ p, const float *__restrict__ g,
                                                  float *__restrict__ m, float *__restrict__ v,
                                                  float *__restrict__ upd, const uint8_t *__restrict__ seg, int64_t P,
                                                  LambC c, const double *__restrict__ sumsq,
                                                  double *__restrict__ seg_sums, const uint32_t *__restrict__ skip) {
    if (skip && *skip) return;
    __shared__ double bins[2 * LAMB_MAX_SEG];
    for (int i = threadIdx.x; i < 2 * LAMB_MAX_SEG; i += blockDim.x) bins[i] = 0.0;
    __syncthreads();
    float coef = c.grad_scale;
    if (sumsq && c.max_norm > 0.f) {
        const float total = (float)sqrt(*sumsq) * fabsf(c.grad_scale);
        coef = c.grad_scale * fminf(c.max_norm / (total + 1e-6f), 1.0f);
    }
    const int64_t tid = (int64_t)blockIdx.x * blockDim.x + threadIdx.x, nt = (int64_t)gridDim.x * blockDim.x;
    for (int64_t i = tid; i < P; i += nt) {
        const int sg = seg[i];
        if (sg >= LAMB_MAX_SEG) continue;
        const float gg = g[i] * coef, w = p[i];
        const float mm = m[i] * c.b1 + c.w1 * gg;
        const float vv = v[i] * c.b2 + c.w2 * (gg * gg);
        m[i] = mm; v[i] = vv;
        const float mh = mm * c.inv_bc1, vh = sqrtf(vv) * c.inv_bc2_sqrt;
        float u = mh / (vh + c.eps);
        if (c.wd > 0.f) u = u + c.wd * w;
        upd[i] = u;
        atomicAdd(&bins[2 * sg], (double)w * (double)w);
        atomicAdd(&bins[2 * sg + 1], (double)u * (double)u);
    }
    __syncthreads();
    for (int i = threadIdx.x; i < 2 * LAMB_MAX_SEG; i += blockDim.x)
        if (bins[i] != 0.0) atomicAdd(&seg_sums[i], bins[i]);
}

__global__ __launch_bounds__(256) void k_lamb_apply(float *__restrict__ p, const float *__restrict__ upd,
                                                    const uint8_t *__restrict__ seg, int64_t P, LambC c,
                                                    const double *__restrict__ seg_sums,
                                                    const uint32_t *__restrict__ skip) {
    if (skip && *skip) return;
    __shared__ float trust[LAMB_MAX_SEG];
    for (int i = threadIdx.x; i < LAMB_MAX_SEG; i += blockDim.x) {
        const float wn = (float)sqrt(seg_sums[2 * i]), sn = (float)sqrt(seg_sums[2 * i + 1]);
        float tr = 1.0f;
        if (c.min_trust != 1.0f && wn != 0.f && sn != 0.f) {
// ... 889 lines not shown
```

### sample_factory_amd/lib.py

```python
from __future__ import annotations

import ctypes as C
import os
import threading
from typing import Optional

import torch

_HERE = os.path.dirname(os.path.abspath(__file__))
LIB_PATH = os.environ.get("SF_HIP_LIB") or os.path.join(_HERE, "libsf_hip.so")


class SfHipError(RuntimeError):
    pass


class sf_loss_cfg(C.Structure):
    _fields_ = [("clip_ratio", C.c_float), ("clip_value", C.c_float), ("value_loss_coeff", C.c_float),
                ("exploration_coeff", C.c_float), ("kl_coeff", C.c_float), ("exploration_kind", C.c_int32),
                ("action_kind", C.c_int32), ("dense_adv", C.c_int32), ("num_heads", C.c_int32),
                ("head_n", C.c_int32 * 8), ("old_values_T", C.c_int32)]


class sf_conv_desc(C.Structure):
    _fields_ = [("Cin", C.c_int32), ("H", C.c_int32), ("W", C.c_int32), ("Cout", C.c_int32), ("KH", C.c_int32),
                ("KW", C.c_int32), ("stride", C.c_int32), ("OH", C.c_int32), ("OW", C.c_int32),
                ("in_u8", C.c_int32), ("relu", C.c_int32), ("traj_T", C.c_int32), ("sub_mean", C.c_float),
                ("inv_scale", C.c_float)]


IN_F32_NHWC, IN_U8_FRAME, IN_F32_FRAME = 0, 1, 2


class sf_res_desc(C.Structure):
    _fields_ = [("Cin", C.c_int32), ("H", C.c_int32), ("W", C.c_int32), ("Cout", C.c_int32), ("in_u8", C.c_int32),
                ("act_in", C.c_int32), ("traj_T", C.c_int32), ("sub_mean", C.c_float), ("inv_scale", C.c_float)]


SYMBOLS = [
    "sf_last_error", "sf_abi_version", "sf_valid_mask", "sf_gae_returns", "sf_moments", "sf_rms_update",
    "sf_rms_apply", "sf_vtrace", "sf_ppo_loss", "sf_loss_scalars", "sf_train_summaries", "sf_minibatch_indices", "sf_minibatch_expand", "sf_grad_sumsq",
    "sf_adam_step", "sf_adam_step_dlr", "sf_lr_kl_adaptive", "sf_clock_probe", "sf_lamb_step", "sf_rnn_cell_fwd", "sf_rnn_cell_bwd", "sf_rows_add_scale", "sf_mlp2_fwd", "sf_rnn_store_state", "sf_rnn_chunk_setup", "sf_lstm_seq_supported", "sf_lstm_seq_fwd", "sf_lstm_seq_bwd", "sf_gru_seq_fwd", "sf_gru_seq_bwd", "sf_seq_fwd_x_supported", "sf_lstm_seq_fwd_x", "sf_gru_seq_fwd_x", "sf_linear_fwd_dual_supported", "sf_linear_fwd_dual",
    "sf_obsnorm_moments", "sf_obsnorm_update", "sf_obsnorm_apply", "sf_sample_write_step",
    "sf_sample_write_step_tuple", "sf_sample_write_step_masked", "sf_traj_write_env_step", "sf_synth_obs",
    "sf_synth_step", "sf_synth_vec_step", "sf_h2d_rows", "sf_copy_rows", "sf_conv_fwd", "sf_conv_fwd_workspace", "sf_conv_wgrad_workspace", "sf_conv_wgrad",
    "sf_conv_dgrad", "sf_conv_norm_supported", "sf_conv_fwd_norm", "sf_conv_wgrad_norm", "sf_conv_relu_mask_supported", "sf_conv_fwd_relu_mask", "sf_conv_wgrad_relu_mask", "sf_conv_kernel_name", "sf_conv_fwd_t_supported", "sf_conv_fwd_t_workspace", "sf_conv_fwd_t", "sf_transpose",
    "sf_tanh_scale_fwd", "sf_tanh_scale_bwd",
    "sf_linear_fwd", "sf_linear_wgrad_workspace", "sf_linear_wgrad", "sf_linear_dgrad", "sf_relu_mask",
    "sf_dp_unique_id", "sf_dp_comm_create", "sf_dp_comm_destroy", "sf_dp_comm_info", "sf_allreduce_grads",
    "sf_dp_allreduce_f64", "sf_dp_broadcast", "sf_dp_oneshot_create", "sf_dp_oneshot_connect", "sf_dp_oneshot_allreduce_f32",
    "sf_dp_oneshot_allreduce_f64", "sf_dp_oneshot_status", "sf_dp_oneshot_destroy",
    "sf_res_conv_fwd", "sf_res_pool_fwd", "sf_res_pool_bwd", "sf_res_conv_dgrad", "sf_res_conv_wgrad_workspace",
    "sf_res_conv_wgrad",
]

_lib: Optional[C.CDLL] = None

_REC = threading.local()
_QUERIES = ("_supported", "_workspace", "_kernel_name", "sf_last_error", "sf_abi_version")
_HOST_STATE = ("sf_h2d_rows", "sf_dp_", "sf_allreduce_grads", "sf_clock_probe")
LAUNCH_PROGRAMS = os.environ.get("SF_LAUNCH_PROGRAMS", "1") != "0"


class LaunchProgram:
    __slots__ = ("calls", "keep", "unsafe")

    def __init__(self):
        self.calls = []
        self.keep = []
        self.unsafe = None

    def replay(self) -> None:
        if PROFILE is None:
            for fn, args, what, _ in self.calls:
                rc = fn(*args)
                if rc:
                    _check(rc, what)
        else:
            for fn, args, what, key in self.calls:
                with _timed(key):
                    _check(fn(*args), what)


class _Recorder:

    def __init__(self, real, prog: LaunchProgram):
        self._real, self.prog, self.key = real, prog, None

    def __getattr__(self, name):
        fn = getattr(self._real, name)
        if name.endswith(_QUERIES):
            return fn
        if name.startswith(_HOST_STATE):
            self.prog.unsafe = self.prog.unsafe or name
            return fn

        def call(*args):
            self.prog.calls.append((fn, args, name, self.key))
            return fn(*args)
        return call


class record_launches:

    def __enter__(self) -> LaunchProgram:
        if getattr(_REC, "rec", None) is not None:
            raise SfHipError("record_launches: already recording on this thread")
        prog = LaunchProgram()
        real = load()
        _REC.rec = _Recorder(real, prog)
        return prog

    def __exit__(self, *a):
        _REC.rec = None
        return False


def recording_unsafe(reason: str) -> None:
    rec = getattr(_REC, "rec", None)
    if rec is not None:
        rec.prog.unsafe = rec.prog.unsafe or reason


def _keep(t):
    rec = getattr(_REC, "rec", None)
# ... 81 lines not shown
                "sample_factory_amd has no CPU/PyTorch fallback for the hot path.")
        lib = C.CDLL(LIB_PATH)
        lib.sf_last_error.restype = C.c_char_p
        lib.sf_conv_wgrad_workspace.restype = C.c_int64
        lib.sf_conv_fwd_workspace.restype = C.c_int64
        lib.sf_conv_fwd_t_workspace.restype = C.c_int64
        lib.sf_linear_wgrad_workspace.restype = C.c_int64
        lib.sf_res_conv_wgrad_workspace.restype = C.c_int64
        _lib = lib
    return _lib


def _check(rc: int, what: str) -> None:
    if rc != 0:
        raise SfHipError(f"{what} failed ({rc}): {load().sf_last_error().decode()}")


_DT = {"f32": torch.float32, "f64": torch.float64, "i32": torch.int32, "u8": (torch.uint8, torch.bool)}


def ptr(t: Optional[torch.Tensor], kind: str, name: str = "tensor") -> C.c_void_p:
    if t is None:
        return C.c_void_p(0)
    want = _DT[kind]
    ok = t.dtype in want if isinstance(want, tuple) else t.dtype == want
    if not ok:
        raise SfHipError(f"{name}: expected dtype {kind}, got {t.dtype}")
    if not t.is_cuda:
        raise SfHipError(f"{name}: tensor lives on {t.device}; the hot path only runs on the GPU (no CPU fallback)")
    if not t.is_contiguous():
        raise SfHipError(f"{name}: tensor must be contiguous (shape {tuple(t.shape)}, strides {t.stride()})")
    return _vp(t)


def _raw(t: torch.Tensor, kind: str, name: str) -> C.c_void_p:
    want = _DT[kind]
    if t.dtype != want:
        raise SfHipError(f"{name}: expected dtype {kind}, got {t.dtype}")
    if not t.is_cuda:
        raise SfHipError(f"{name}: tensor lives on {t.device}; the hot path only runs on the GPU (no CPU fallback)")
    return _vp(t)


def stream() -> C.c_void_p:
    return C.c_void_p(torch.cuda.current_stream().cuda_stream)


def f(x) -> C.c_float:
    return x if isinstance(x, C.c_float) else C.c_float(float(x))


def i64(x) -> C.c_int64:
    return C.c_int64(int(x))


def u32(x) -> C.c_uint32:
    return x if isinstance(x, C.c_uint32) else C.c_uint32(int(x) & 0xFFFFFFFF)


def valid_mask(policy_id, policy_version, valids, actions, num_actions, log_prob_actions, my_policy_id, train_step,
               max_policy_lag, num_invalid, valids_flat=None) -> None:
    E, T = policy_id.shape
    if valids_flat is not None and valids_flat.numel() != E * T:
        raise SfHipError(f"valid_mask: valids_flat must hold E*T = {E * T} elements, got {valids_flat.numel()}")
    _check(load().sf_valid_mask(ptr(policy_id, "i32", "policy_id"), ptr(policy_version, "f32", "policy_version"),
                                ptr(valids, "u8", "valids"), ptr(valids_flat, "u8", "valids_flat"),
                                ptr(actions, "f32", "actions"), int(num_actions),
                                ptr(log_prob_actions, "f32", "log_prob_actions"), E, T, int(my_policy_id),
                                int(train_step), int(max_policy_lag), ptr(num_invalid, "i32", "num_invalid"),
                                stream()), "sf_valid_mask")


def gae_returns(rewards, dones, time_outs, values, valids, rms_stats, gamma, gae_lambda, value_bootstrap, advantages,
                returns) -> None:
    E, T = rewards.shape
    assert values.shape == (E, T + 1) and valids.shape == (E, T + 1)
    _check(load().sf_gae_returns(ptr(rewards, "f32", "rewards"), ptr(dones, "u8", "dones"),
                                 ptr(time_outs, "u8", "time_outs"), ptr(values, "f32", "values"),
                                 ptr(valids, "u8", "valids"), ptr(rms_stats, "f64", "rms_stats"), E, T, f(gamma),
                                 f(gae_lambda), int(bool(value_bootstrap)), ptr(advantages, "f32", "advantages"),
                                 ptr(returns, "f32", "returns"), stream()), "sf_gae_returns")


def moments(x, valids, index, n, out, offset=0, dense_x=False) -> None:
    _check(load().sf_moments(ptr(x, "f32", "x"), ptr(valids, "u8", "valids"), ptr(index, "i32", "index"), i64(offset),
                             i64(n), int(bool(dense_x)), ptr(out, "f64", "moments"), stream()), "sf_moments")


def rms_update(stats_in, mom, stats_out) -> None:
    _check(load().sf_rms_update(ptr(stats_in, "f64"), ptr(mom, "f64"), ptr(stats_out, "f64"), stream()),
           "sf_rms_update")


def rms_apply(x, stats, denormalize: bool) -> None:
    _check(load().sf_rms_apply(ptr(x, "f32", "x"), i64(x.numel()), ptr(stats, "f64"), int(bool(denormalize)),
                               stream()), "sf_rms_apply")


def _raw_any(t: torch.Tensor, u8: bool, name: str) -> C.c_void_p:
    want = torch.uint8 if u8 else torch.float32
    if t.dtype != want:
        raise SfHipError(f"{name}: expected {want}, got {t.dtype}")
    if not t.is_cuda:
        raise SfHipError(f"{name} lives on {t.device}; the hot path only runs on the GPU (no CPU fallback)")
    return _vp(t)


def obsnorm_moments(inp, u8, stride, index, offset, traj_T, n, D, sub_mean, inv_scale, s, ss) -> None:
    _check(load().sf_obsnorm_moments(_raw_any(inp, u8, "obs"), int(u8), i64(stride), ptr(index, "i32", "index"),
                                     i64(offset), int(traj_T), i64(n), int(D), f(sub_mean), f(inv_scale),
                                     ptr(s, "f64", "sum"), ptr(ss, "f64", "sumsq"), stream()), "sf_obsnorm_moments")


def obsnorm_update(mean, var, count_in, count_out, s, ss, n, D, mu_tab, rstd_tab) -> None:
    _check(load().sf_obsnorm_update(ptr(mean, "f64"), ptr(var, "f64"), ptr(count_in, "f64"), ptr(count_out, "f64"),
                                    ptr(s, "f64"), ptr(ss, "f64"), i64(n), int(D), ptr(mu_tab, "f32"),
                                    ptr(rstd_tab, "f32"), stream()), "sf_obsnorm_update")


def obsnorm_apply(inp, u8, stride, index, offset, traj_T, n, D, C_, HW, sub_mean, inv_scale, mu, rstd, out) -> None:
    _check(load().sf_obsnorm_apply(_raw_any(inp, u8, "obs"), int(u8), i64(stride), ptr(index, "i32", "index"),
                                   i64(offset), int(traj_T), i64(n), int(D), int(C_), int(HW), f(sub_mean),
                                   f(inv_scale), ptr(mu, "f32"), ptr(rstd, "f32"), ptr(out, "f32", "out"), stream()),
           "sf_obsnorm_apply")


def _rp(t, name="tensor"):
    return C.c_void_p(0) if t is None else _raw(t, "f32", name)


def rnn_cell_fwd(kind, gx, gh, h_prev, ld_h, c_prev, ld_c, keep, Cn, H, gates_out, h_out, c_out, h_next, c_next) -> None:
    _check(load().sf_rnn_cell_fwd(int(kind), ptr(gx, "f32", "gx"), ptr(gh, "f32", "gh"), _rp(h_prev, "h_prev"),
                                  i64(ld_h), _rp(c_prev, "c_prev"), i64(ld_c), ptr(keep, "f32", "keep"), int(Cn),
                                  int(H), ptr(gates_out, "f32"), ptr(h_out, "f32"), ptr(c_out, "f32"),
                                  ptr(h_next, "f32"), ptr(c_next, "f32"), stream()), "sf_rnn_cell_fwd")


def rnn_cell_bwd(kind, dh, dc_in, gates, h_prev, ld_h, c_prev, ld_c, c_out, Cn, H, dgx, dgh, dh_direct, dc_prev) -> None:
    _check(load().sf_rnn_cell_bwd(int(kind), ptr(dh, "f32", "dh"), ptr(dc_in, "f32"), ptr(gates, "f32", "gates"),
                                  _rp(h_prev, "h_prev"), i64(ld_h), _rp(c_prev, "c_prev"), i64(ld_c),
                                  ptr(c_out, "f32"), int(Cn), int(H), ptr(dgx, "f32", "dgx"), ptr(dgh, "f32"),
                                  ptr(dh_direct, "f32"), ptr(dc_prev, "f32"), stream()), "sf_rnn_cell_bwd")


def mlp2_supported(D, H1, H2) -> bool:
    return (H1 % 8 == 0 and H2 % 8 == 0 and (D * H1 + H1 * H2 + 64 * (D + H1)) * 4 <= 64 * 1024 and D <= 64 and
            D * H1 <= 8192 and H1 * H2 <= 8192)


def mlp2_fwd(x, x_stride, n, D, sub_mean, inv_scale, mu, rstd, w1, b1, w2, b2, act, out) -> None:
    _check(load().sf_mlp2_fwd(_raw(x, "f32", "x"), i64(x_stride), i64(n), int(D), f(sub_mean), f(inv_scale),
                              ptr(mu, "f32", "mu"), ptr(rstd, "f32", "rstd"), ptr(w1, "f32", "w1"), ptr(b1, "f32", "b1"),
                              int(w1.shape[1]), ptr(w2, "f32", "w2"), ptr(b2, "f32", "b2"), int(w2.shape[1]), int(act),
                              ptr(out, "f32", "out"), stream()), "sf_mlp2_fwd")


def rnn_store_state(h, c, dones_col, out) -> None:
    B, H = h.shape
    if dones_col.dtype not in (torch.bool, torch.uint8) or not dones_col.is_cuda or dones_col.shape != (B,):
        raise SfHipError(f"rnn_store_state: dones must be a device bool/u8 [B] column, got {dones_col.dtype} {tuple(dones_col.shape)}")
    if out.shape != (B, H if c is None else 2 * H) or out.stride(1) != 1:
        raise SfHipError(f"rnn_store_state: out must be [B, {H if c is None else 2 * H}] with unit column stride")
    _check(load().sf_rnn_store_state(ptr(h, "f32", "h"), ptr(c, "f32", "c"), _vp(dones_col),
                                     i64(dones_col.stride(0)), _raw(out, "f32", "out"), i64(out.stride(0)), i64(B), int(H),
                                     stream()), "sf_rnn_store_state")


def rnn_chunk_setup(dones, valids, rnn_states, index, offset, Cn, R, keep_tm, h0, traj_T=0) -> None:
    S = rnn_states.shape[-1]
# ... 40 lines not shown
               "sf_lstm_seq_fwd")


def lstm_seq_bwd(dout, gates, cprev, cout, keep, whh, dgx, sync, R, Cn, H, env_major=False) -> None:
    with _timed(_seq_key("lstm_bwd", R, Cn, H, R - 1)):
        _check(load().sf_lstm_seq_bwd(ptr(dout, "f32", "dout"), ptr(gates, "f32", "gates"), ptr(cprev, "f32", "cprev"),
                                      ptr(cout, "f32", "cout"), ptr(keep, "f32", "keep"), ptr(whh, "f32", "whh"),
                                      ptr(dgx, "f32", "dgx"),
                                      ptr(sync, "i32", "sync"), int(R), int(Cn), int(H), int(bool(env_major)), stream()),
               "sf_lstm_seq_bwd")


def gru_seq_fwd(gx, whh, bhh, keep, gates, hprev, hout, sync, R, Cn, H, env_major=False) -> None:
    with _timed(_seq_key("gru_fwd", R, Cn, H, R, 3)):
        _check(load().sf_gru_seq_fwd(ptr(gx, "f32", "gx"), ptr(whh, "f32", "whh"), ptr(bhh, "f32", "bhh"),
                                     ptr(keep, "f32", "keep"), ptr(gates, "f32", "gates"), ptr(hprev, "f32", "hprev"),
                                     ptr(hout, "f32", "hout"), ptr(sync, "i32", "sync"), int(R), int(Cn), int(H),
                                     int(bool(env_major)), stream()), "sf_gru_seq_fwd")


def linear_fwd_dual_supported(n: int, N: int, K1: int, K2: int) -> bool:
    return bool(load().sf_linear_fwd_dual_supported(i64(n), int(N), int(K1), int(K2)))


def linear_fwd_dual(a1, lda1, w1t, bias1, a2, lda2, w2t, bias2, out, n, gru_H=0) -> None:
    N, K1, K2 = int(out.shape[1]), int(w1t.shape[1]), int(w2t.shape[1])
    key = None if not _keys_wanted() else ("fwd_dual", int(n), K1 + K2, 1, 1, 3 * int(gru_H) if gru_H else N, 1, 1, 1, 1, "k_fwd_glds2<128, 64, 2, 2>")
    with _timed(key):
        _check(load().sf_linear_fwd_dual(_raw(a1, "f32", "a1"), i64(lda1), ptr(w1t, "f32", "w1t"), ptr(bias1, "f32", "bias1"), K1,
                                         _raw(a2, "f32", "a2"), i64(lda2), ptr(w2t, "f32", "w2t"), ptr(bias2, "f32", "bias2"), K2,
                                         ptr(out, "f32", "out"), i64(n), N, int(gru_H), stream()), "sf_linear_fwd_dual")


def seq_fwd_x_supported(Cn: int, H: int, Kx: int) -> bool:
    return bool(load().sf_seq_fwd_x_supported(int(Cn), int(H), int(Kx)))


def lstm_seq_fwd_x(x, wih_t, bih, whh, bhh, keep, gates, hprev, hout, cprev, cout, sync, R, Cn, H, env_major=False) -> None:
    Kx = int(wih_t.shape[1])
    with _timed(_seq_key("lstm_fwd", R, Cn, H, R, x_cols=Kx)):
        _check(load().sf_lstm_seq_fwd_x(ptr(x, "f32", "x"), ptr(wih_t, "f32", "wih_t"), ptr(bih, "f32", "bih"), Kx,
                                        ptr(whh, "f32", "whh"), ptr(bhh, "f32", "bhh"), ptr(keep, "f32", "keep"),
                                        ptr(gates, "f32", "gates"), ptr(hprev, "f32", "hprev"), ptr(hout, "f32", "hout"),
                                        ptr(cprev, "f32", "cprev"), ptr(cout, "f32", "cout"), ptr(sync, "i32", "sync"),
                                        int(R), int(Cn), int(H), int(bool(env_major)), stream()), "sf_lstm_seq_fwd_x")


def gru_seq_fwd_x(x, wih_t, bih, whh, bhh, keep, gates, hprev, hout, sync, R, Cn, H, env_major=False) -> None:
    Kx = int(wih_t.shape[1])
    with _timed(_seq_key("gru_fwd", R, Cn, H, R, 3, x_cols=Kx)):
        _check(load().sf_gru_seq_fwd_x(ptr(x, "f32", "x"), ptr(wih_t, "f32", "wih_t"), ptr(bih, "f32", "bih"), Kx,
                                       ptr(whh, "f32", "whh"), ptr(bhh, "f32", "bhh"), ptr(keep, "f32", "keep"),
                                       ptr(gates, "f32", "gates"), ptr(hprev, "f32", "hprev"), ptr(hout, "f32", "hout"),
                                       ptr(sync, "i32", "sync"), int(R), int(Cn), int(H), int(bool(env_major)), stream()),
               "sf_gru_seq_fwd_x")


def gru_seq_bwd(dout, gates, hprev, keep, whh, dgx, dgh, sync, R, Cn, H, env_major=False) -> None:
    with _timed(_seq_key("gru_bwd", R, Cn, H, R - 1, 3)):
        _check(load().sf_gru_seq_bwd(ptr(dout, "f32", "dout"), ptr(gates, "f32", "gates"), ptr(hprev, "f32", "hprev"),
                                     ptr(keep, "f32", "keep"), ptr(whh, "f32", "whh"), ptr(dgx, "f32", "dgx"),
                                     ptr(dgh, "f32", "dgh"), ptr(sync, "i32", "sync"), int(R), int(Cn), int(H),
                                     int(bool(env_major)), stream()), "sf_gru_seq_bwd")


def rows_add_scale(a, b, keep, Cn, H, y) -> None:
    _check(load().sf_rows_add_scale(ptr(a, "f32", "a"), ptr(b, "f32"), ptr(keep, "f32"), i64(Cn), int(H),
                                    ptr(y, "f32", "y"), stream()), "sf_rows_add_scale")


def vtrace(params, ld_params, values, ld_values, actions, old_logp, rewards, dones, index, offset, n, A, action_kind,
           recurrence, gamma, rho_hat, c_hat, vs, adv, head_sizes=None) -> None:
    hn = (C.c_int32 * 8)(*[int(x) for x in head_sizes]) if head_sizes and len(head_sizes) > 1 else None
    _check(load().sf_vtrace(_raw(params, "f32", "params"), int(ld_params), _raw(values, "f32", "values"),
                            int(ld_values), ptr(actions, "f32", "actions"),
                            ptr(old_logp, "f32", "old_logp"), ptr(rewards, "f32", "rewards"), ptr(dones, "u8", "dones"),
                            ptr(index, "i32", "index"), i64(offset), i64(n), int(A), int(action_kind),
                            int(recurrence), f(gamma), f(rho_hat), f(c_hat), ptr(vs, "f32", "vs"),
                            ptr(adv, "f32", "adv"), hn, len(head_sizes) if hn is not None else 0, stream()),
           "sf_vtrace")


def ppo_loss(params, ld_params, values, ld_values, actions, old_logp, old_params, old_values, adv, targets, valids,
             index, offset, n, A, cfg: sf_loss_cfg, mom, sums, g_params, g_values, ratio_out=None) -> None:
    _check(load().sf_ppo_loss(_raw(params, "f32", "params"), int(ld_params), _raw(values, "f32", "values"),
                              int(ld_values), ptr(actions, "f32", "actions"), ptr(old_logp, "f32", "old_logp"),
                              ptr(old_params, "f32", "old_params"), ptr(old_values, "f32", "old_values"),
                              ptr(adv, "f32", "adv"), ptr(targets, "f32", "targets"), ptr(valids, "u8", "valids"),
                              ptr(index, "i32", "index"), i64(offset), i64(n), int(A), C.byref(cfg),
                              ptr(mom, "f64", "moments"), ptr(sums, "f64", "sums"), _raw(g_params, "f32", "g_params"),
                              _raw(g_values, "f32", "g_values"), ptr(ratio_out, "f32", "ratio_out"), stream()),
           "sf_ppo_loss")


def loss_scalars(sums, mom, cfg: sf_loss_cfg, out) -> None:
    _check(load().sf_loss_scalars(ptr(sums, "f64"), ptr(mom, "f64"), C.byref(cfg), ptr(out, "f32"), stream()),
           "sf_loss_scalars")


def train_summaries(valids, ratio, values, ld_values, old_values, old_values_T, actions, num_actions, adv, dense_adv,
                    policy_id, policy_version, action_logits, A, index, offset, n, my_policy_id, train_step, clip_ratio,
                    exp_avg_sq, out) -> None:
    _check(load().sf_train_summaries(ptr(valids, "u8", "valids"), ptr(ratio, "f32", "ratio"), _raw(values, "f32", "values"),
                                     int(ld_values), ptr(old_values, "f32", "old_values"), int(old_values_T),
                                     ptr(actions, "f32", "actions"), int(num_actions), ptr(adv, "f32", "adv"),
                                     int(bool(dense_adv)), ptr(policy_id, "i32", "policy_id"),
                                     ptr(policy_version, "f32", "policy_version"), ptr(action_logits, "f32", "action_logits"),
                                     int(A), ptr(index, "i32", "index"), i64(offset), i64(n), int(my_policy_id),
                                     int(train_step), f(clip_ratio), ptr(exp_avg_sq, "f32", "exp_avg_sq"),
                                     i64(exp_avg_sq.numel() if exp_avg_sq is not None else 0), ptr(out, "f64", "out"),
                                     stream()), "sf_train_summaries")


def minibatch_indices(out, experience_size, recurrence, shuffle, seed, epoch) -> None:
    _check(load().sf_minibatch_indices(ptr(out, "i32", "indices"), i64(experience_size), int(recurrence),
                                       int(bool(shuffle)), u32(seed), u32(epoch), stream()), "sf_minibatch_indices")


def minibatch_expand(chunk_starts, out, experience_size, recurrence) -> None:
    _check(load().sf_minibatch_expand(ptr(chunk_starts, "i32", "chunk_starts"), ptr(out, "i32", "out"),
                                      i64(experience_size), int(recurrence), stream()), "sf_minibatch_expand")


def grad_sumsq(g, sumsq) -> None:
    _check(load().sf_grad_sumsq(ptr(g, "f32", "grad"), i64(g.numel()), ptr(sumsq, "f64", "sumsq"), stream()),
           "sf_grad_sumsq")


def adam_step(p, g, m, v, step, lr, beta1, beta2, eps, max_grad_norm, sumsq, grad_scale=1.0, skip_flag=None) -> None:
    _check(load().sf_adam_step(ptr(p, "f32", "params"), ptr(g, "f32", "grads"), ptr(m, "f32", "exp_avg"),
                               ptr(v, "f32", "exp_avg_sq"), i64(p.numel()), int(step), f(lr), f(beta1), f(beta2),
                               f(eps), f(max_grad_norm), ptr(sumsq, "f64", "sumsq"), f(grad_scale),
                               ptr(skip_flag, "i32", "skip_flag"), stream()),
           "sf_adam_step")


def adam_step_dlr(p, g, m, v, step, lr_dev, lr_scale, beta1, beta2, eps, max_grad_norm, sumsq, grad_scale=1.0,
                  skip_flag=None) -> None:
    _check(load().sf_adam_step_dlr(ptr(p, "f32", "params"), ptr(g, "f32", "grads"), ptr(m, "f32", "exp_avg"),
                                   ptr(v, "f32", "exp_avg_sq"), i64(p.numel()), int(step), ptr(lr_dev, "f32", "lr_dev"),
                                   f(lr_scale), f(beta1), f(beta2), f(eps), f(max_grad_norm), ptr(sumsq, "f64", "sumsq"),
                                   f(grad_scale), ptr(skip_flag, "i32", "skip_flag"), stream()), "sf_adam_step_dlr")


def lr_kl_adaptive(kl, lr_dev, threshold, lr_min, lr_max, lr_out=None) -> None:
    _check(load().sf_lr_kl_adaptive(ptr(kl, "f32", "kl"), ptr(lr_dev, "f32", "lr_dev"), f(threshold), f(lr_min), f(lr_max),
                                    ptr(lr_out, "f32", "lr_out"), stream()), "sf_lr_kl_adaptive")


def clock_probe(out: torch.Tensor, spin_cycles: int = 200000, on_stream=None) -> None:
    if not out.is_cuda or out.dtype != torch.int64 or out.numel() < 2:
        raise SfHipError("clock_probe: out must be a device int64 tensor of 2 elements")
    st = C.c_void_p(on_stream.cuda_stream) if on_stream is not None else stream()
    _check(load().sf_clock_probe(C.c_void_p(out.data_ptr()), int(spin_cycles), st), "sf_clock_probe")


def lamb_step(p, g, m, v, scratch, seg_id, seg_sums, num_segments, step, lr, beta1, beta2, eps, weight_decay, min_trust,
              max_grad_norm, sumsq, grad_scale=1.0, skip_flag=None) -> None:
    _check(load().sf_lamb_step(ptr(p, "f32", "p"), ptr(g, "f32", "g"), ptr(m, "f32", "m"), ptr(v, "f32", "v"),
                               ptr(scratch, "f32", "scratch"), ptr(seg_id, "u8", "seg_id"), ptr(seg_sums, "f64", "seg_sums"),
                               i64(p.numel()), int(num_segments), int(step), f(lr), f(beta1), f(beta2), f(eps),
                               f(weight_decay), f(min_trust), f(max_grad_norm), ptr(sumsq, "f64", "sumsq"),
                               f(grad_scale), ptr(skip_flag, "i32", "skip_flag"), stream()), "sf_lamb_step")


def sample_write_step(logits, ld_logits, values, ld_values, B, A, T, t, seed, step, row0, policy_version, deterministic,
                      traj_actions, traj_logits, traj_logp, traj_values, traj_policy_version, env_actions,
                      action_kind=0) -> None:
    _check(load().sf_sample_write_step(_raw(logits, "f32", "logits"), int(ld_logits), _raw(values, "f32", "values"),
                                       int(ld_values), int(B), int(A), int(T),
                                       int(t), u32(seed), u32(step), u32(row0), f(policy_version),
                                       int(bool(deterministic)), int(action_kind), ptr(traj_actions, "f32"),
                                       ptr(traj_logits, "f32"),
                                       ptr(traj_logp, "f32"), ptr(traj_values, "f32"),
                                       ptr(traj_policy_version, "f32"), ptr(env_actions, "i32"), stream()),
           "sf_sample_write_step")


def sample_write_step_masked(logits, ld_logits, values, ld_values, mask, ld_mask, B, A, T, t, seed, step, row0,
                             policy_version, deterministic, traj_actions, traj_logits, traj_logp, traj_values,
                             traj_policy_version, env_actions) -> None:
    if mask.dtype not in (torch.uint8, torch.bool) or not mask.is_cuda:
        raise SfHipError(f"action_mask: expected a u8/bool CUDA tensor, got {mask.dtype} on {mask.device}")
    _check(load().sf_sample_write_step_masked(_raw(logits, "f32", "logits"), int(ld_logits),
                                              _raw(values, "f32", "values"), int(ld_values),
                                              _vp(mask), i64(ld_mask), int(B), int(A), int(T), int(t),
                                              u32(seed), u32(step), u32(row0), f(policy_version),
                                              int(bool(deterministic)), ptr(traj_actions, "f32"),
                                              ptr(traj_logits, "f32"), ptr(traj_logp, "f32"), ptr(traj_values, "f32"),
                                              ptr(traj_policy_version, "f32"), ptr(env_actions, "i32"), stream()),
           "sf_sample_write_step_masked")


def sample_write_step_tuple(logits, ld_logits, values, ld_values, B, head_n, T, t, seed, step, row0, policy_version,
                            deterministic, traj_actions, traj_logits, traj_logp, traj_values, traj_policy_version,
                            env_actions) -> None:
    hn = (C.c_int32 * 8)(*[int(x) for x in head_n])
    _check(load().sf_sample_write_step_tuple(_raw(logits, "f32", "logits"), int(ld_logits),
                                             _raw(values, "f32", "values"), int(ld_values), int(B), len(head_n), hn,
                                             int(T), int(t), u32(seed), u32(step), u32(row0), f(policy_version),
                                             int(bool(deterministic)), ptr(traj_actions, "f32"), ptr(traj_logits, "f32"),
                                             ptr(traj_logp, "f32"), ptr(traj_values, "f32"),
                                             ptr(traj_policy_version, "f32"), ptr(env_actions, "i32"), stream()),
           "sf_sample_write_step_tuple")


def traj_write_env_step(rewards, terminated, truncated, T, t, reward_scale, reward_clip, policy_id, traj_rewards,
                        traj_dones, traj_time_outs, traj_policy_id, ep_return, ep_len, ep_stats) -> None:
    B = rewards.numel()
    _check(load().sf_traj_write_env_step(ptr(rewards, "f32", "rewards"), ptr(terminated, "u8", "terminated"),
                                         ptr(truncated, "u8", "truncated"), B, int(T), int(t), f(reward_scale),
                                         f(reward_clip), int(policy_id), ptr(traj_rewards, "f32"),
                                         ptr(traj_dones, "u8"), ptr(traj_time_outs, "u8"), ptr(traj_policy_id, "i32"),
                                         ptr(ep_return, "f32"), ptr(ep_len, "i32"), ptr(ep_stats, "f64"), stream()),
           "sf_traj_write_env_step")


def synth_vec_step(state, actions, obs_out, env0, seed, step, reset, rewards, terminated) -> None:
    B, D = state.shape
    A = actions.shape[1] if actions is not None else 0
    _check(load().sf_synth_vec_step(
        ptr(state, "f32", "state"), _raw(actions, "f32", "actions") if actions is not None else C.c_void_p(0),
        i64(actions.stride(0) if actions is not None else 0), _raw(obs_out, "f32", "obs_out"), i64(obs_out.stride(0)),
        int(B), int(D), int(A), int(env0), u32(seed), u32(step), int(bool(reset)),
        ptr(rewards, "f32", "rewards"), ptr(terminated, "u8", "terminated"), stream()), "sf_synth_vec_step")
# ... 328 lines not shown
```

### sample_factory_amd/model/actor_critic.py

```python
from __future__ import annotations

import math
import threading
from typing import Dict, List, Optional

import numpy as np
import torch

from sample_factory_amd import lib
from sample_factory_amd.algo.utils.running_mean_std import RunningMeanStdInPlace
from sample_factory_amd.envs.spaces import is_box, calc_num_action_parameters

import os

_LSTM_SEQ = os.environ.get("SF_LSTM_SEQ", "1") != "0"
_CONV1_NORM = os.environ.get("SF_CONV1_NORM", "1") != "0"
_MLP2 = os.environ.get("SF_MLP2", "1") != "0"

ACT_KIND = {"relu": 1, "tanh": 2, "elu": 3}
FRAME_KINDS = {"conv_u8": lib.IN_U8_FRAME, "conv_f32frame": lib.IN_F32_FRAME}

CONV_ARCHS = {
    "convnet_simple": [[32, 8, 4], [64, 4, 2], [128, 3, 2]],
    "convnet_impala": [[16, 8, 4], [32, 4, 2]],
# ... 24 lines not shown
        self.role = role
        self.in_act_kind = 0
        self.rnn_l = 0
        self.desc = desc
        self.kind = kind
        self.ref_w_shape = ref_w_shape
        self.first_fc_chw = first_fc_chw
        self.K = desc.KH * desc.KW * desc.Cin
        self.N = desc.Cout
        self.w = self.b = self.gw = self.gb = self.wt = None

    @property
    def out_pixels(self):
        return self.desc.OH * self.desc.OW

    def w_from_ref(self, w_ref: torch.Tensor) -> torch.Tensor:
        d = self.desc
        if self.kind in FRAME_KINDS:
            return w_ref.reshape(d.Cout, self.K).t().contiguous()
        if self.kind == "conv":
            return w_ref.permute(2, 3, 1, 0).reshape(self.K, d.Cout).contiguous()
        if self.kind == "linear_after_conv":
            C, OH, OW = self.first_fc_chw
            return w_ref.view(self.N, C, OH, OW).permute(2, 3, 1, 0).reshape(self.K, self.N).contiguous()
        return w_ref.t().contiguous()

    def w_to_ref(self, w: torch.Tensor) -> torch.Tensor:
        d = self.desc
        if self.kind in FRAME_KINDS:
            return w.t().reshape(d.Cout, d.Cin, d.KH, d.KW).contiguous()
        if self.kind == "conv":
            return w.reshape(d.KH, d.KW, d.Cin, d.Cout).permute(3, 2, 0, 1).contiguous()
        if self.kind == "linear_after_conv":
            C, OH, OW = self.first_fc_chw
            return w.reshape(OH, OW, C, self.N).permute(3, 2, 0, 1).reshape(self.N, self.K).contiguous()
        return w.t().contiguous()


def _linear_desc(K, N, relu) -> lib.sf_conv_desc:
    return lib.sf_conv_desc(Cin=K, H=1, W=1, Cout=N, KH=1, KW=1, stride=1, OH=1, OW=1, in_u8=0, relu=int(relu),
                            traj_T=0, sub_mean=0.0, inv_scale=1.0)


class NativeModel:

    def eval(self):
        return self.train(False)

    def model_to_device(self, device):
        assert torch.device(device).type == "cuda", "the native model only lives on the GPU"

    def normalize_obs(self, obs):
        return obs


class NativeTower(NativeModel):

    def _init_scratch(self) -> None:
        self._bufs: Dict = {}
        self._layout_gen = 0
        self._wss: Dict = {}
        self._tls = threading.local()
        self._snap = None
        self._snap_tabs = None
        self.snap_read = 0

    def _buf(self, key, shape, dtype=torch.float32):
        t = self._bufs.get(key)
        if t is None or t.shape != torch.Size(shape) or t.dtype != dtype:
            t = torch.empty(shape, dtype=dtype, device=self.device)
            self._bufs[key] = t
            self._layout_gen += 1
        return t

    def _zbuf(self, key, shape):
        t = self._bufs.get(key)
        if t is None or t.shape != torch.Size(shape):
            t = torch.zeros(shape, dtype=torch.float32, device=self.device)
            self._bufs[key] = t
            self._layout_gen += 1
        return t

    def _workspace(self, nbytes: int) -> torch.Tensor:
        key = getattr(self._tls, "role", "learner")
        ws = self._wss.get(key)
        if ws is None or ws.numel() < nbytes:
            ws = torch.empty(max(int(nbytes), 16), dtype=torch.uint8, device=self.device)
            self._wss[key] = ws
            self._layout_gen += 1
        return ws

    def launch_key(self, tag: str = "inf"):
        return (self._layout_gen, self.snap_read if self._snap is not None else -1)

    @property
    def _norm_prefix(self) -> str:
        return f"obs_normalizer.running_mean_std.running_mean_std.{self.obs_key}."

    def normalizer_state(self) -> Dict[str, torch.Tensor]:
        return self.obs_normalizer.state_dict(self._norm_prefix) if self.obs_normalizer is not None else {}

    def load_normalizer_state(self, sd) -> None:
        if self.obs_normalizer is not None and self._norm_prefix + "count" in sd:
            self.obs_normalizer.load_state_dict(sd, self._norm_prefix)

    def initialize_weights(self):
        cfg = self.cfg
        gain = cfg.policy_init_gain
        sd = {}
        for name, shape in self.ref_param_shapes():
            t = torch.empty(shape, dtype=torch.float32)
            if name.endswith("learned_stddev"):
                t.fill_(math.log(cfg.initial_stddev))
            elif name.startswith("core.core."):
                bound = 1.0 / math.sqrt(self.rnn_H)
                t.uniform_(-bound, bound)
            elif name.endswith(".bias"):
                if cfg.policy_initialization == "torch_default":
                    fan_in = int(np.prod(dict(self.ref_param_shapes())[name[:-4] + "weight"][1:]))
                    bound = 1 / math.sqrt(fan_in)
                    t.uniform_(-bound, bound)
                else:
                    t.zero_()
            elif cfg.policy_initialization == "orthogonal":
                torch.nn.init.orthogonal_(t, gain=gain)
            elif cfg.policy_initialization == "xavier_uniform":
                torch.nn.init.xavier_uniform_(t, gain=gain)
            else:
                torch.nn.init.kaiming_uniform_(t, a=math.sqrt(5))
            sd[name] = t
        self.load_state_dict(sd, strict=False)


class ActorCritic(NativeTower):

    def __init__(self, cfg, obs_space, action_space, device="cuda", all_reduce=None, obs_key: str = "obs", part: str = "full"):
        assert part in ("full", "encoder", "trunk")
        self.cfg = cfg
        self.obs_space = obs_space
        self.action_space = action_space
        self.device = torch.device(device)
        self.training = True
        self.part, self.obs_key = part, obs_key
        self.headless, self.features_in = part == "encoder", part == "trunk"
        self.g_input = None
        if cfg.use_rnn and (cfg.rnn_num_layers < 1 or cfg.rnn_type not in ("gru", "lstm")):
            raise NotImplementedError("native recurrent core: GRU or LSTM, rnn_num_layers >= 1")
        if not cfg.actor_critic_share_weights:
            raise NotImplementedError("separate actor/critic weights: model/actor_critic_separate.py composes two towers")
        if cfg.nonlinearity not in ACT_KIND:
            raise NotImplementedError(f"Unknown nonlinearity {cfg.nonlinearity}")
        act = ACT_KIND[cfg.nonlinearity]
        keys_ = getattr(cfg, "normalize_input_keys", None)
        norm_input = bool(cfg.normalize_input) and (not keys_ or obs_key in keys_) and not self.features_in
        self.nonadaptive_std = is_box(action_space) and not cfg.adaptive_stddev and not self.headless
        self.tanh_scale = float(cfg.continuous_tanh_scale) if self.nonadaptive_std else 0.0
        keys = sorted(k for k in obs_space.spaces.keys() if k != "action_mask")
        if part != "encoder" and keys != ["obs"]:
            raise NotImplementedError(f"single 'obs' key (+ optional 'action_mask') only, got {keys}")
        space = obs_space[obs_key]
        self.obs_shape = tuple(space.shape)
        self.obs_u8 = np.dtype(space.dtype) == np.uint8
        self.obs_f32 = np.dtype(space.dtype) == np.float32
        self.num_action_params = calc_num_action_parameters(action_space)
        self.layers: List[_Layer] = []
        sub_mean = float(cfg.obs_subtract_mean)
        inv_scale = float(np.float32(1.0 / cfg.obs_scale)) if abs(cfg.obs_scale - 1.0) > 1e-5 else 1.0
        if abs(sub_mean) <= 1e-5:
            sub_mean = 0.0
        if obs_key != "obs" or self.features_in:
            sub_mean, inv_scale = 0.0, 1.0

        self._fused_norm = False
# ... 528 lines not shown
        return torch.cat([t for h, c in self._rnn_out[tag] for t in ((h,) if c is None else (h, c))], dim=1)

    @property
    def new_rnn_states(self) -> torch.Tensor:
        return self.new_rnn_states_of("inf")

    def _seq_sync_buf(self) -> torch.Tensor:
        t = self._bufs.get(("rnn", "seq_sync"))
        if t is None:
            t = self._bufs[("rnn", "seq_sync")] = torch.zeros(192, dtype=torch.int32, device=self.device)
        return t

    def rnn_abort_word(self) -> Optional[torch.Tensor]:
        return self._seq_sync_buf()[128:129] if (self.rnn_kind is not None and _LSTM_SEQ) else None

    def rnn_abort_clear(self) -> None:
        if self.rnn_kind is not None and _LSTM_SEQ:
            self._seq_sync_buf()[128:129].zero_()

    def rnn_pass_aborted(self) -> bool:
        t = self._bufs.get(("rnn", "seq_sync"))
        return t is not None and bool(int(t[128].item()))

    def forward(self, normalized_obs_dict, rnn_states=None, values_only: bool = False, action_mask=None):
        obs = normalized_obs_dict["obs"] if isinstance(normalized_obs_dict, dict) else normalized_obs_dict
        B = obs.shape[0]
        rnn = dict(states=rnn_states) if self.rnn_kind is not None else None
        heads = self.forward_heads(obs, B, sample_stride=self.obs_elems if obs.is_contiguous() else obs.stride(0),
                                   rnn=rnn)[-1]
        res = dict(values=heads[:, 0])
        if not values_only:
            res["action_logits"] = heads[:, 1:1 + self.num_action_params]
        res["new_rnn_states"] = self.new_rnn_states if self.rnn_kind is not None else rnn_states
        return res

    def backward(self, acts: List[torch.Tensor], g_heads: torch.Tensor, obs: torch.Tensor, n: int, *,
                 sample_stride: int, index=None, offset: int = 0, traj_T: int = 0, on_layer_done=None) -> None:
        ctx = self._ctx["train"]
        self._tls.role = "learner"
        inputs = ctx["inputs"]
        x0, stride0, idx0, off0, tT0 = ctx["first_in"]
        g = g_heads
        if self.tanh_scale > 0:
            lib.tanh_scale_bwd(g_heads, ctx["acts"][-1], self.heads_ld, n, 1, self.num_action_params // 2, self.tanh_scale)
        chain = [li for li, L in enumerate(self.layers) if L.role != "rnn_hh"]
        mask0 = ctx.get("relu_mask0")
        for pos in range(len(chain) - 1, -1, -1):
            li = chain[pos]
            L = self.layers[li]
            d = L.desc
            if L.role == "rnn_ih":
                g = self._rnn_sequence_bwd(li, g, n)
            if pos == 0 and not self.features_in:
                d0 = lib.sf_conv_desc.from_buffer_copy(d)
                d0.traj_T = int(tT0)
                ws = self._workspace(lib.conv_wgrad_workspace(n, d0))
                if ctx.get("norm_tabs") is not None:
                    mu_, rstd_ = ctx["norm_tabs"]
                    lib.conv_wgrad_norm(x0, stride0, idx0, off0, mu_, rstd_, g, L.gw, L.gb, n, d0, ws)
                elif mask0 is not None:
                    lib.conv_wgrad_relu_mask(x0, stride0, idx0, off0, g, mask0, L.gw, L.gb, n, d0, ws)
                else:
                    lib.conv_wgrad_raw(x0, stride0, idx0, off0, g, L.gw, L.gb, n, d0, ws)
            else:
                x = inputs[li]
                ws = self._workspace(lib.conv_wgrad_workspace(n, d))
                lib.conv_wgrad_raw(x, d.H * d.W * d.Cin, None, 0, g, L.gw, L.gb, n, d, ws)
                gin = self._buf(("g", li - 1), tuple(x.shape))
                dd = lib.sf_conv_desc.from_buffer_copy(d)
                dd.relu = L.in_act_kind
                if pos == 1 and mask0 is not None:
                    dd.relu = 0
                    lib.conv_dgrad(g, L.w, None, gin, n, dd)
                else:
                    lib.conv_dgrad(g, L.w, x if L.in_act_kind else None, gin, n, dd)
                g = gin
                if L.role == "rnn_ih":
                    R, Cn = self._rnn_saved["R"], self._rnn_saved["Cn"]
                    gs = self._buf(("g", "x_sm", li), (n, L.K))
                    gs.view(Cn, R, L.K).copy_(g.view(R, Cn, L.K).transpose(0, 1))
                    g = gs
                if pos == 0:
                    self.g_input = g
            if self.nonadaptive_std and li == len(self.layers) - 1:
                A = self.num_action_params
                L.gw[:, 1 + A // 2:1 + A].zero_()
            if on_layer_done is not None:
                on_layer_done(li)
```

Before: 2.106 million.

## Batch backward partial reductions and fuse grad-norm, transpose and loss-buffer clears into tail kernels

```diff
diff --git a/include/sf_hip.h b/include/sf_hip.h
--- a/include/sf_hip.h
+++ b/include/sf_hip.h
@@ -71,6 +71,14 @@
                 float *ratio_out ,
                 void *stream);
 int sf_loss_scalars(const double *sums, const double *moments, const sf_loss_cfg *h_cfg, float *out, void *stream);
+int sf_moments_acc(const float *x, const uint8_t *valids, const int32_t *index, int64_t offset, int64_t n, int dense_x,
+                   double *moments, void *stream);
+int sf_ppo_loss_acc(const float *params, int ld_params, const float *values, int ld_values, const float *actions,
+                    const float *old_logp, const float *old_params, const float *old_values, const float *adv,
+                    const float *targets, const uint8_t *valids, const int32_t *index, int64_t offset, int64_t n, int A,
+                    const sf_loss_cfg *h_cfg, const double *moments, double *sums, float *g_params, float *g_values,
+                    float *ratio_out, void *stream);
+int sf_loss_scalars_clear(double *sums, double *moments, const sf_loss_cfg *h_cfg, float *out, void *stream);
 int sf_train_summaries(const uint8_t *valids, const float *ratio, const float *values, int ld_values,
                        const float *old_values, int old_values_T, const float *actions, int num_actions, const float *adv,
                        int dense_adv, const int32_t *policy_id, const float *policy_version, const float *action_logits,
@@ -91,6 +99,17 @@
                      float grad_scale, const uint32_t *skip_flag, void *stream);
 int sf_lr_kl_adaptive(const float *kl, float *lr_dev, float threshold, float lr_min, float lr_max, float *lr_out,
                       void *stream);
+#define SF_ADAM_MAX_WT 8
+typedef struct sf_adam_wt_tab {
+    int32_t count;
+    int32_t K[SF_ADAM_MAX_WT], N[SF_ADAM_MAX_WT];
+    int32_t reserved_;
+    int64_t offset[SF_ADAM_MAX_WT];
+} sf_adam_wt_tab;
+int sf_adam_step_wt(float *p, const float *g, float *m, float *v, float *pt, int64_t P, int step, float lr,
+                    const float *lr_dev, float beta1, float beta2, float eps, float max_grad_norm, const double *sumsq,
+                    float grad_scale, const uint32_t *skip_flag, const sf_adam_wt_tab *tab, double *zero_after,
+                    void *stream);
 int sf_clock_probe(unsigned long long *out, int spin_cycles, void *stream);
 
 int sf_lamb_step(float *p, const float *g, float *m, float *v, float *scratch, const uint8_t *seg_id, double *seg_sums,
@@ -152,6 +171,13 @@
 int64_t sf_conv_wgrad_workspace(int64_t n, const sf_conv_desc *h_desc);
 int sf_conv_wgrad(const void *in, int64_t in_sample_stride, const int32_t *index, int64_t offset, const float *dout,
                   float *dw, float *db, int64_t n, const sf_conv_desc *h_desc, void *workspace, void *stream);
+#define SF_REDUCE_MAX_JOBS 16
+int sf_reduce_jobs_create(void **tab);
+int sf_reduce_jobs_destroy(void *tab);
+int sf_reduce_defer_begin(void *tab, double *sumsq);
+int sf_reduce_jobs_add(void *tab, const float *partial, float *out, int64_t n, int Z, void *stream);
+int sf_reduce_partials_batch(void *tab, const float *grads, int64_t P, void *stream);
+int sf_reduce_partials(const float *partial, float *out, int64_t n, int Z, void *stream);
 int sf_conv_dgrad(const float *dout, const float *w, const float *in_act, float *din, int64_t n,
                   const sf_conv_desc *h_desc, void *stream);
 int sf_conv_relu_mask_supported(int64_t n, const sf_conv_desc *h_desc);
diff --git a/sample_factory_amd/algo/learning/learner.py b/sample_factory_amd/algo/learning/learner.py
--- a/sample_factory_amd/algo/learning/learner.py
+++ b/sample_factory_amd/algo/learning/learner.py
@@ -181,6 +181,17 @@
         self._moments = torch.zeros(3, dtype=torch.float64, device=dev)
         self._sums = torch.zeros(8, dtype=torch.float64, device=dev)
         self._sumsq = torch.zeros(1, dtype=torch.float64, device=dev)
+        ft = lib.fuse_tail()
+        plain = type(ac_) is ActorCritic and not self.dp
+        self._fuse_reduce = lib.ReduceJobs() if plain and ft & 1 else None
+        self._fuse_norm = (self._fuse_reduce is not None and bool(ft & 2) and cfg.optimizer == "adam" and
+                           not ac_.nonadaptive_std)
+        self._adam_wt = ac_.adam_wt_table() if plain and ft & 4 and cfg.optimizer == "adam" else None
+        self._arena = torch.zeros(16, dtype=torch.float64, device=dev) if plain and ft & 8 else None
+        if self._arena is not None:
+            self._sums, self._moments = self._arena[0:8], self._arena[8:11]
+        self._sumsq2 = torch.zeros(2, dtype=torch.float64, device=dev)
+        self._norm_slot = 0
         self._scalars = None
         A = calc_num_action_parameters(self.env_info.action_space)
         self.num_action_params = A
@@ -423,6 +434,7 @@
         cfg, ac = self.cfg, self.actor_critic
         index, offset, n = mb
         A = self.num_action_params
+        arena = self._arena is not None and moments is None
         rnn = None
         if cfg.use_rnn:
             R, Cn = cfg.recurrence, n // cfg.recurrence
@@ -442,10 +454,10 @@
             lib.vtrace(params, ld, values, ld, buff.actions, buff.log_prob_actions, buff.rewards, buff.dones, index,
                        offset, n, A, self.loss_cfg.action_kind, cfg.recurrence, cfg.gamma, cfg.vtrace_rho,
                        cfg.vtrace_c, vs, adv, head_sizes=self._head_sizes)
-            lib.moments(adv, buff.valids, index, n, self._moments, offset=offset, dense_x=True)
+            lib.moments(adv, buff.valids, index, n, self._moments, offset=offset, dense_x=True, acc=arena)
             adv_arr, tgt_arr = adv, vs
         elif moments is None:
-            lib.moments(buff.advantages, buff.valids, index, n, self._moments, offset=offset)
+            lib.moments(buff.advantages, buff.valids, index, n, self._moments, offset=offset, acc=arena)
             adv_arr, tgt_arr = buff.advantages, buff.returns
         else:
             adv_arr, tgt_arr = buff.advantages, buff.returns
@@ -456,12 +468,12 @@
         self.loss_cfg.old_values_T = buff.T
         lib.ppo_loss(params, ld, values, ld, buff.actions, buff.log_prob_actions, buff.action_logits, buff["values"],
                      adv_arr, tgt_arr, buff.valids, index, offset, n, A, self.loss_cfg, moments, self._sums,
-                     g_heads[:, 1:], g_heads[:, 0], ratio_out=self._ratio)
+                     g_heads[:, 1:], g_heads[:, 0], ratio_out=self._ratio, acc=arena)
         self._last_mb = (index, offset, n, values, adv_arr)
         if self.dp and self._dp_reduce_each_mb:
             self.group.loss_sums(self._sums)
         out = scalars_out if scalars_out is not None else torch.zeros(16, dtype=torch.float32, device=self.device)
-        lib.loss_scalars(self._sums, moments, self.loss_cfg, out)
+        lib.loss_scalars(self._sums, moments, self.loss_cfg, out, clear=arena)
         return acts, g_heads, out
 
     def _epoch_moments(self, buff: AttrDict, minibatches) -> Optional[torch.Tensor]:
@@ -490,6 +502,9 @@
                 self._lr_dev = torch.zeros(1, dtype=torch.float32, device=self.device)
             self._lr_dev.fill_(float(self.curr_lr))
         self._grad_norms = []
+        if self._arena is not None:
+            self._arena.zero_()
+        fused_norm = self._fuse_norm and (cfg.max_grad_norm > 0.0 or getattr(cfg, "record_grad_norm", False))
         skip = ac.rnn_abort_word() if hasattr(ac, "rnn_abort_word") else None
         if skip is not None:
             ac.rnn_abort_clear()
@@ -511,6 +526,16 @@
                     self.group.all_reduce_grads(ac.flat_grads[:cut])
                     for work in pending:
                         work.wait()
+                elif self._fuse_reduce is not None:
+                    if fused_norm:
+                        self._norm_slot ^= 1
+                        self._sumsq = self._sumsq2[self._norm_slot:self._norm_slot + 1]
+                    ac.defer_reductions(self._fuse_reduce, self._sumsq if fused_norm else None)
+                    try:
+                        ac.backward(acts, g_heads, buff.obs, n, sample_stride=ac.obs_elems, index=index, offset=offset,
+                                    traj_T=buff.T)
+                    finally:
+                        ac.run_reductions(fused_norm)
                 else:
                     ac.backward(acts, g_heads, buff.obs, n, sample_stride=ac.obs_elems, index=index, offset=offset,
                                 traj_T=buff.T)
@@ -524,7 +549,8 @@
                 self.adam_step_count += 1
                 use_clip = cfg.max_grad_norm > 0.0
                 if use_clip or getattr(cfg, "record_grad_norm", False):
-                    lib.grad_sumsq(ac.flat_grads, self._sumsq)
+                    if not fused_norm:
+                        lib.grad_sumsq(ac.flat_grads, self._sumsq)
                     if getattr(cfg, "record_grad_norm", False):
                         self._grad_norms.append(float(self._sumsq.sqrt().item()))
                 if cfg.optimizer == "lamb":
@@ -537,17 +563,25 @@
                                   nseg, self.adam_step_count, actual_lr, cfg.adam_beta1, cfg.adam_beta2, cfg.adam_eps,
                                   1e-4, 0.01, cfg.max_grad_norm if use_clip else 0.0, self._sumsq if use_clip else None,
                                   skip_flag=skip)
-                elif lr_on_device:
-                    lib.adam_step_dlr(ac.flat_params, ac.flat_grads, self.exp_avg, self.exp_avg_sq, self.adam_step_count,
-                                      self._lr_dev, valid_frac, cfg.adam_beta1, cfg.adam_beta2, cfg.adam_eps,
+                else:
+                    wt = {}
+                    if fused_norm or self._adam_wt is not None:
+                        other = self._norm_slot ^ 1
+                        wt = dict(pt=ac.flat_params_t,
+                                  wt_tab=self._adam_wt if self._adam_wt is not None else lib.sf_adam_wt_tab(),
+                                  zero_after=self._sumsq2[other:other + 1] if fused_norm else None)
+                    if lr_on_device:
+                        lib.adam_step_dlr(ac.flat_params, ac.flat_grads, self.exp_avg, self.exp_avg_sq, self.adam_step_count,
+                                          self._lr_dev, valid_frac, cfg.adam_beta1, cfg.adam_beta2, cfg.adam_eps,
+                                          cfg.max_grad_norm if use_clip else 0.0, self._sumsq if use_clip else None,
+                                          skip_flag=skip, **wt)
+                    else:
+                        lib.adam_step(ac.flat_params, ac.flat_grads, self.exp_avg, self.exp_avg_sq, self.adam_step_count,
+                                      actual_lr, cfg.adam_beta1, cfg.adam_beta2, cfg.adam_eps,
                                       cfg.max_grad_norm if use_clip else 0.0, self._sumsq if use_clip else None,
-                                      skip_flag=skip)
-                else:
-                    lib.adam_step(ac.flat_params, ac.flat_grads, self.exp_avg, self.exp_avg_sq, self.adam_step_count,
-                                  actual_lr, cfg.adam_beta1, cfg.adam_beta2, cfg.adam_eps,
-                                  cfg.max_grad_norm if use_clip else 0.0, self._sumsq if use_clip else None,
-                                  skip_flag=skip)
-                ac.params_changed()
+                                      skip_flag=skip, **wt)
+                if self._adam_wt is None:
+                    ac.params_changed()
                 num_sgd_steps += 1
                 self.train_step += 1
                 if lr_on_device:
diff --git a/sample_factory_amd/csrc/sf_nn.hip b/sample_factory_amd/csrc/sf_nn.hip
--- a/sample_factory_amd/csrc/sf_nn.hip
+++ b/sample_factory_amd/csrc/sf_nn.hip
@@ -611,12 +611,179 @@
     if (zg == 0 && i < n)
         out[i] = ((sm[0][li] + sm[1][li]) + (sm[2][li] + sm[3][li])) + ((sm[4][li] + sm[5][li]) + (sm[6][li] + sm[7][li]));
 }
-static void launch_reduce_partials(const float *partial, float *out, int64_t n, int Z, hipStream_t st) {
+static bool reduce_takes_tree(int64_t n, int Z) {
     static const int tree_on = getenv("SF_REDUCE_TREE") ? atoi(getenv("SF_REDUCE_TREE")) : 1;
-    if (tree_on && Z >= 64 && (n + 255) / 256 < 256)
+    return tree_on && Z >= 64 && (n + 255) / 256 < 256;
+}
+
+enum { RJ_TREE = 0, RJ_LOOP = 1, RJ_SQUARE = 2 };
+struct ReduceJob {
+    const float *partial;
+    float *out;
+    int64_t n;
+    int Z, kind, blk0, nblk;
+};
+struct ReduceBatch {
+    ReduceJob job[SF_REDUCE_MAX_JOBS];
+    int count;
+};
+
+__global__ __launch_bounds__(256) void k_reduce_partials_batch(ReduceBatch b, double *__restrict__ sumsq) {
+    __shared__ float sm[8][33];
+    __shared__ double lds[4];
+    int j = 0;
+    while (j + 1 < b.count && (int)blockIdx.x >= b.job[j + 1].blk0) ++j;
+    const float *__restrict__ partial = b.job[j].partial;
+    float *__restrict__ out = b.job[j].out;
+    const int64_t n = b.job[j].n;
+    const int Z = b.job[j].Z, kind = b.job[j].kind, bx = (int)blockIdx.x - b.job[j].blk0, nblk = b.job[j].nblk;
+    double sq[1] = {0.0};
+    if (kind == RJ_TREE) {
+        const int li = threadIdx.x & 31, zg = threadIdx.x >> 5;
+        const int64_t i = (int64_t)bx * 32 + li;
+        const int zper = (Z + 7) / 8, z0 = zg * zper, z1 = z0 + zper < Z ? z0 + zper : Z;
+        float s[8] = {0.f, 0.f, 0.f, 0.f, 0.f, 0.f, 0.f, 0.f};
+        if (i < n) {
+            int z = z0;
+            for (; z + 8 <= z1; z += 8) {
+#pragma unroll
+                for (int q = 0; q < 8; ++q) s[q] += partial[(int64_t)(z + q) * n + i];
+            }
+            for (int q = 0; z < z1; ++z, ++q) s[q] += partial[(int64_t)z * n + i];
+        }
+        sm[zg][li] = ((s[0] + s[1]) + (s[2] + s[3])) + ((s[4] + s[5]) + (s[6] + s[7]));
+        __syncthreads();
+        if (zg == 0 && i < n) {
+            const float r = ((sm[0][li] + sm[1][li]) + (sm[2][li] + sm[3][li])) + ((sm[4][li] + sm[5][li]) + (sm[6][li] + sm[7][li]));
+            out[i] = r;
+            sq[0] = (double)r * r;
+        }
+    } else if (kind == RJ_LOOP) {
+        for (int64_t i = (int64_t)bx * blockDim.x + threadIdx.x; i < n; i += (int64_t)nblk * blockDim.x) {
+            float s[8] = {0.f, 0.f, 0.f, 0.f, 0.f, 0.f, 0.f, 0.f};
+            int z = 0;
+            for (; z + 8 <= Z; z += 8) {
+#pragma unroll
+                for (int q = 0; q < 8; ++q) s[q] += partial[(int64_t)(z + q) * n + i];
+            }
+            for (int q = 0; z < Z; ++z, ++q) s[q] += partial[(int64_t)z * n + i];
+            const float r = ((s[0] + s[1]) + (s[2] + s[3])) + ((s[4] + s[5]) + (s[6] + s[7]));
+            out[i] = r;
+            sq[0] += (double)r * r;
+        }
+    } else {
+        for (int64_t i = (int64_t)bx * blockDim.x + threadIdx.x; i < n; i += (int64_t)nblk * blockDim.x)
+            sq[0] += (double)partial[i] * partial[i];
+    }
+    if (sumsq) {
+        sf_block_sum<1>(sq, lds);
+        if (threadIdx.x == 0) atomicAdd(sumsq, sq[0]);
+    }
+}
+
+struct ReduceTable {
+    ReduceBatch b;
+    double *sumsq;
+    int ncov, cov_lost;
+    const float *cov_lo[64], *cov_hi[64];
+};
+static thread_local ReduceTable *tl_defer = nullptr;
+
+static int reduce_table_flush(ReduceTable *t, hipStream_t st) {
+    if (t->b.count == 0) return SF_OK;
+    int blocks = 0;
+    for (int j = 0; j < t->b.count; ++j) {
+        t->b.job[j].blk0 = blocks;
+        blocks += t->b.job[j].nblk;
+    }
+    k_reduce_partials_batch<<<dim3((unsigned)blocks), dim3(256), 0, st>>>(t->b, t->sumsq);
+    t->b.count = 0;
+    return sf_launch_status("sf_reduce_partials_batch");
+}
+
+static int reduce_table_add(ReduceTable *t, const float *partial, float *out, int64_t n, int Z, int kind, hipStream_t st) {
+    if (t->b.count == SF_REDUCE_MAX_JOBS) {
+        const int rc = reduce_table_flush(t, st);
+        if (rc) return rc;
+    }
+    ReduceJob &J = t->b.job[t->b.count++];
+    J.partial = partial; J.out = out; J.n = n; J.Z = Z; J.kind = kind; J.blk0 = 0;
+    if (kind == RJ_TREE) J.nblk = (int)((n + 31) / 32);
+    else if (kind == RJ_LOOP) J.nblk = (int)((n + 255) / 256 < 2048 ? (n + 255) / 256 : 2048);
+    else J.nblk = (int)((n + 255) / 256 < 256 ? (n + 255) / 256 : 256);
+    if (kind != RJ_SQUARE) {
+        if (t->ncov < 64) { t->cov_lo[t->ncov] = out; t->cov_hi[t->ncov] = out + n; ++t->ncov; }
+        else t->cov_lost = 1;
+    }
+    return SF_OK;
+}
+
+static int launch_reduce_partials(const float *partial, float *out, int64_t n, int Z, hipStream_t st) {
+    if (tl_defer) return reduce_table_add(tl_defer, partial, out, n, Z, reduce_takes_tree(n, Z) ? RJ_TREE : RJ_LOOP, st);
+    if (reduce_takes_tree(n, Z))
         k_reduce_partials_tree<<<dim3((unsigned)((n + 31) / 32)), dim3(256), 0, st>>>(partial, out, n, Z);
     else
         k_reduce_partials<<<dim3((unsigned)((n + 255) / 256 < 2048 ? (n + 255) / 256 : 2048)), dim3(256), 0, st>>>(partial, out, n, Z);
+    return SF_OK;
+}
+
+extern "C" int sf_reduce_jobs_create(void **tab) {
+    SF_REQUIRE(tab, "sf_reduce_jobs_create: null pointer");
+    ReduceTable *t = (ReduceTable *)calloc(1, sizeof(ReduceTable));
+    SF_REQUIRE(t, "sf_reduce_jobs_create: out of host memory");
+    *tab = t;
+    return SF_OK;
+}
+extern "C" int sf_reduce_jobs_destroy(void *tab) {
+    if (tl_defer == tab) tl_defer = nullptr;
+    free(tab);
+    return SF_OK;
+}
+extern "C" int sf_reduce_defer_begin(void *tab, double *sumsq) {
+    SF_REQUIRE(tab, "sf_reduce_defer_begin: null table");
+    ReduceTable *t = (ReduceTable *)tab;
+    SF_REQUIRE(t->b.count == 0, "sf_reduce_defer_begin: the table still holds %d jobs (sf_reduce_partials_batch runs them)", t->b.count);
+    t->sumsq = sumsq;
+    t->ncov = t->cov_lost = 0;
+    tl_defer = t;
+    return SF_OK;
+}
+extern "C" int sf_reduce_jobs_add(void *tab, const float *partial, float *out, int64_t n, int Z, void *stream) {
+    SF_REQUIRE(tab && partial && out && n > 0 && Z > 0, "sf_reduce_jobs_add: bad args");
+    return reduce_table_add((ReduceTable *)tab, partial, out, n, Z, reduce_takes_tree(n, Z) ? RJ_TREE : RJ_LOOP, STREAM(stream));
+}
+extern "C" int sf_reduce_partials_batch(void *tab, const float *grads, int64_t P, void *stream) {
+    SF_REQUIRE(tab && P >= 0, "sf_reduce_partials_batch: bad args");
+    ReduceTable *t = (ReduceTable *)tab;
+    if (tl_defer == t) tl_defer = nullptr;
+    if (grads && P > 0 && t->sumsq) {
+        SF_REQUIRE(!t->cov_lost, "sf_reduce_partials_batch: more than 64 reductions since sf_reduce_defer_begin; take the norm with sf_grad_sumsq");
+        const float *at = grads, *end = grads + P;
+        bool used[64] = {false};
+        for (;;) {
+            int best = -1;
+            for (int c = 0; c < t->ncov; ++c)
+                if (!used[c] && t->cov_hi[c] > at && t->cov_lo[c] < end && (best < 0 || t->cov_lo[c] < t->cov_lo[best])) best = c;
+            const float *lo = best < 0 ? end : t->cov_lo[best];
+            if (lo > at) {
+                const int rc = reduce_table_add(t, at, nullptr, lo - at, 0, RJ_SQUARE, STREAM(stream));
+                if (rc) return rc;
+            }
+            if (best < 0) break;
+            used[best] = true;
+            if (t->cov_hi[best] > at) at = t->cov_hi[best];
+            if (at >= end) break;
+        }
+    }
+    return reduce_table_flush(t, STREAM(stream));
+}
+extern "C" int sf_reduce_partials(const float *partial, float *out, int64_t n, int Z, void *stream) {
+    SF_REQUIRE(partial && out && n > 0 && Z > 0, "sf_reduce_partials: bad args");
+    ReduceTable *keep = tl_defer;
+    tl_defer = nullptr;
+    launch_reduce_partials(partial, out, n, Z, STREAM(stream));
+    tl_defer = keep;
+    return sf_launch_status("sf_reduce_partials");
 }
 
 template <int BM, int BN, int WM, int WN, bool VEC>
diff --git a/sample_factory_amd/csrc/sf_rl.hip b/sample_factory_amd/csrc/sf_rl.hip
--- a/sample_factory_amd/csrc/sf_rl.hip
+++ b/sample_factory_amd/csrc/sf_rl.hip
@@ -205,15 +205,23 @@
     }
 }
 
-extern "C" int sf_moments(const float *x, const uint8_t *valids, const int32_t *index, int64_t offset, int64_t n,
-                          int dense_x, double *moments, void *stream) {
+static int moments_impl(const float *x, const uint8_t *valids, const int32_t *index, int64_t offset, int64_t n,
+                        int dense_x, double *moments, bool clear, void *stream) {
     SF_REQUIRE(x && moments && n >= 0 && offset >= 0, "sf_moments: bad args");
-    int rc = sf_hip_status(hipMemsetAsync(moments, 0, 3 * sizeof(double), STREAM(stream)), "sf_moments memset");
+    int rc = clear ? sf_hip_status(hipMemsetAsync(moments, 0, 3 * sizeof(double), STREAM(stream)), "sf_moments memset") : 0;
     if (rc || n == 0) return rc;
     const int64_t blocks = (n + 255) / 256;
     k_moments<<<dim3((unsigned)(blocks < 2048 ? blocks : 2048)), dim3(256), 0, STREAM(stream)>>>(
         x, valids, index, offset, n, dense_x, moments);
     return sf_launch_status("sf_moments");
+}
+extern "C" int sf_moments(const float *x, const uint8_t *valids, const int32_t *index, int64_t offset, int64_t n,
+                          int dense_x, double *moments, void *stream) {
+    return moments_impl(x, valids, index, offset, n, dense_x, moments, true, stream);
+}
+extern "C" int sf_moments_acc(const float *x, const uint8_t *valids, const int32_t *index, int64_t offset, int64_t n,
+                              int dense_x, double *moments, void *stream) {
+    return moments_impl(x, valids, index, offset, n, dense_x, moments, false, stream);
 }
 
 __global__ void k_rms_update(const double *__restrict__ stats_in, const double *__restrict__ moments,
@@ -826,12 +834,12 @@
     return h;
 }
 
-extern "C" int sf_ppo_loss(const float *params, int ld_params, const float *values, int ld_values,
-                           const float *actions, const float *old_logp, const float *old_params,
-                           const float *old_values, const float *adv, const float *targets, const uint8_t *valids,
-                           const int32_t *index, int64_t offset, int64_t n, int A, const sf_loss_cfg *h_cfg,
-                           const double *moments, double *sums, float *g_params, float *g_values, float *ratio_out,
-                           void *stream) {
+static int ppo_loss_impl(const float *params, int ld_params, const float *values, int ld_values,
+                         const float *actions, const float *old_logp, const float *old_params,
+                         const float *old_values, const float *adv, const float *targets, const uint8_t *valids,
+                         const int32_t *index, int64_t offset, int64_t n, int A, const sf_loss_cfg *h_cfg,
+                         const double *moments, double *sums, float *g_params, float *g_values, float *ratio_out,
+                         bool clear, void *stream) {
     SF_REQUIRE(ld_params >= A && ld_values >= 1, "sf_ppo_loss: bad strides");
     SF_REQUIRE(params && values && actions && old_logp && old_params && old_values && adv && targets && valids &&
                    h_cfg && moments && sums && g_params && g_values,
@@ -841,7 +849,7 @@
     SF_REQUIRE(!(h_cfg->exploration_kind == 2 && h_cfg->action_kind != 0 && h_cfg->exploration_coeff != 0.f),
                "sf_ppo_loss: symmetric_kl exploration loss needs a categorical distribution");
     const LossDev h = make_loss_dev(h_cfg);
-    int rc = sf_hip_status(hipMemsetAsync(sums, 0, 8 * sizeof(double), STREAM(stream)), "sf_ppo_loss memset");
+    int rc = clear ? sf_hip_status(hipMemsetAsync(sums, 0, 8 * sizeof(double), STREAM(stream)), "sf_ppo_loss memset") : 0;
     if (rc) return rc;
     const dim3 grid((unsigned)((n + 255) / 256)), block(256);
 #define PL_DISPATCH(KERNEL, ...)                                                        \
@@ -883,10 +891,26 @@
 #undef PL_DISPATCH
     return sf_launch_status("sf_ppo_loss");
 }
-
-__global__ void k_loss_scalars(const double *__restrict__ sums, const double *__restrict__ moments, LossDev h,
-                               float *__restrict__ out) {
-    if (threadIdx.x || blockIdx.x) return;
+extern "C" int sf_ppo_loss(const float *params, int ld_params, const float *values, int ld_values,
+                           const float *actions, const float *old_logp, const float *old_params,
+                           const float *old_values, const float *adv, const float *targets, const uint8_t *valids,
+                           const int32_t *index, int64_t offset, int64_t n, int A, const sf_loss_cfg *h_cfg,
+                           const double *moments, double *sums, float *g_params, float *g_values, float *ratio_out,
+                           void *stream) {
+    return ppo_loss_impl(params, ld_params, values, ld_values, actions, old_logp, old_params, old_values, adv, targets, valids,
+                         index, offset, n, A, h_cfg, moments, sums, g_params, g_values, ratio_out, true, stream);
+}
+extern "C" int sf_ppo_loss_acc(const float *params, int ld_params, const float *values, int ld_values,
+                               const float *actions, const float *old_logp, const float *old_params,
+                               const float *old_values, const float *adv, const float *targets, const uint8_t *valids,
+                               const int32_t *index, int64_t offset, int64_t n, int A, const sf_loss_cfg *h_cfg,
+                               const double *moments, double *sums, float *g_params, float *g_values, float *ratio_out,
+                               void *stream) {
+    return ppo_loss_impl(params, ld_params, values, ld_values, actions, old_logp, old_params, old_values, adv, targets, valids,
+                         index, offset, n, A, h_cfg, moments, sums, g_params, g_values, ratio_out, false, stream);
+}
+
+__device__ __forceinline__ void loss_scalars1(const double *sums, const double *moments, const LossDev &h, float *out) {
     const double n = moments[2];
     const double mean64 = moments[0] / n;
     const double var64 = (moments[1] - moments[0] * mean64) / (n - 1.0);
@@ -906,12 +930,28 @@
     out[8] = (float)n;
     out[9] = (float)(sums[1] / n);
 }
+__global__ void k_loss_scalars(const double *__restrict__ sums, const double *__restrict__ moments, LossDev h,
+                               float *__restrict__ out) {
+    if (threadIdx.x || blockIdx.x) return;
+    loss_scalars1(sums, moments, h, out);
+}
+__global__ void k_loss_scalars_clear(double *sums, double *moments, LossDev h, float *__restrict__ out) {
+    if (threadIdx.x || blockIdx.x) return;
+    loss_scalars1(sums, moments, h, out);
+    for (int i = 0; i < 8; ++i) sums[i] = 0.0;
+    for (int i = 0; i < 3; ++i) moments[i] = 0.0;
+}
 
 extern "C" int sf_loss_scalars(const double *sums, const double *moments, const sf_loss_cfg *h_cfg, float *out,
                                void *stream) {
     SF_REQUIRE(sums && moments && h_cfg && out, "sf_loss_scalars: null pointer");
     k_loss_scalars<<<dim3(1), dim3(64), 0, STREAM(stream)>>>(sums, moments, make_loss_dev(h_cfg), out);
     return sf_launch_status("sf_loss_scalars");
+}
+extern "C" int sf_loss_scalars_clear(double *sums, double *moments, const sf_loss_cfg *h_cfg, float *out, void *stream) {
+    SF_REQUIRE(sums && moments && h_cfg && out, "sf_loss_scalars_clear: null pointer");
+    k_loss_scalars_clear<<<dim3(1), dim3(64), 0, STREAM(stream)>>>(sums, moments, make_loss_dev(h_cfg), out);
+    return sf_launch_status("sf_loss_scalars_clear");
 }
 
 constexpr int SUMM_NS = 8, SUMM_NM = 11, SUMM_OUT = 24;
@@ -1265,6 +1305,119 @@
     SF_REQUIRE(lr_dev, "sf_adam_step_dlr: null lr_dev");
     return adam_step_impl(p, g, m, v, P, step, lr_scale, beta1, beta2, eps, max_grad_norm, sumsq, grad_scale, skip_flag,
                           lr_dev, stream, "sf_adam_step_dlr");
+}
+
+struct AdamWtPlan {
+    int64_t off[SF_ADAM_MAX_WT], plo[SF_ADAM_MAX_WT + 1], phi[SF_ADAM_MAX_WT + 1];
+    int K[SF_ADAM_MAX_WT], N[SF_ADAM_MAX_WT], tile0[SF_ADAM_MAX_WT + 1];
+    int nwt, nplain;
+};
+
+__global__ __launch_bounds__(256) void k_adam_wt(float *__restrict__ p, const float *__restrict__ g,
+                                                 float *__restrict__ m, float *__restrict__ v, float *__restrict__ pt,
+                                                 AdamC c, const double *__restrict__ sumsq,
+                                                 const uint32_t *__restrict__ skip, const float *__restrict__ lr_dev,
+                                                 AdamWtPlan t, double *__restrict__ zero_after) {
+    __shared__ float tile[32][33];
+    if (zero_after && blockIdx.x == 0 && threadIdx.x == 0) *zero_after = 0.0;
+    if (skip && *skip) return;
+    if (lr_dev) c.lr_step *= *lr_dev;
+    float coef = c.grad_scale;
+    if (sumsq && c.max_norm > 0.f) {
+        const float total = (float)sqrt(*sumsq) * fabsf(c.grad_scale);
+        const float cc = c.max_norm / (total + 1e-6f);
+        coef = c.grad_scale * fminf(cc, 1.0f);
+    }
+    const int ntile = t.tile0[t.nwt];
+    if ((int)blockIdx.x < ntile) {
+        int l = 0;
+        while (l + 1 < t.nwt && (int)blockIdx.x >= t.tile0[l + 1]) ++l;
+        const int K = t.K[l], N = t.N[l], tb = (int)blockIdx.x - t.tile0[l], ntn = (N + 31) / 32;
+        const int k0 = (tb / ntn) * 32, n0 = (tb % ntn) * 32, cc_ = threadIdx.x & 31, r0 = threadIdx.x >> 5;
+        const int64_t off = t.off[l];
+#pragma unroll
+        for (int j = 0; j < 4; ++j) {
+            const int r = r0 + 8 * j, k = k0 + r, n = n0 + cc_;
+            if (k < K && n < N) {
+                const int64_t e = off + (int64_t)k * N + n;
+                float pp = p[e], mm = m[e], vv = v[e];
+                adam1(pp, g[e], mm, vv, c, coef);
+                p[e] = pp; m[e] = mm; v[e] = vv;
+                tile[r][cc_] = pp;
+            }
+        }
+        __syncthreads();
+#pragma unroll
+        for (int j = 0; j < 4; ++j) {
+            const int r = r0 + 8 * j, n = n0 + r, k = k0 + cc_;
+            if (n < N && k < K) pt[off + (int64_t)n * K + k] = tile[cc_][r];
+        }
+        return;
+    }
+    const int64_t tid = (int64_t)((int)blockIdx.x - ntile) * blockDim.x + threadIdx.x;
+    const int64_t nt = (int64_t)((int)gridDim.x - ntile) * blockDim.x;
+    for (int s = 0; s < t.nplain; ++s) {
+        const int64_t lo = t.plo[s], hi = t.phi[s];
+        const int64_t a4 = (lo + 3) / 4 * 4 < hi ? (lo + 3) / 4 * 4 : hi, b4 = hi / 4 * 4 > a4 ? hi / 4 * 4 : a4;
+        for (int64_t i = lo + tid; i < a4; i += nt) adam1(p[i], g[i], m[i], v[i], c, coef);
+        float4 *p4 = reinterpret_cast<float4 *>(p), *m4 = reinterpret_cast<float4 *>(m), *v4 = reinterpret_cast<float4 *>(v);
+        const float4 *g4 = reinterpret_cast<const float4 *>(g);
+        for (int64_t i = a4 / 4 + tid; i < b4 / 4; i += nt) {
+            float4 pp = p4[i], mm = m4[i], vv = v4[i];
+            const float4 gg = g4[i];
+            adam1(pp.x, gg.x, mm.x, vv.x, c, coef);
+            adam1(pp.y, gg.y, mm.y, vv.y, c, coef);
+            adam1(pp.z, gg.z, mm.z, vv.z, c, coef);
+            adam1(pp.w, gg.w, mm.w, vv.w, c, coef);
+            p4[i] = pp; m4[i] = mm; v4[i] = vv;
+        }
+        for (int64_t i = b4 + tid; i < hi; i += nt) adam1(p[i], g[i], m[i], v[i], c, coef);
+    }
+}
+
+extern "C" int sf_adam_step_wt(float *p, const float *g, float *m, float *v, float *pt, int64_t P, int step, float lr,
+                               const float *lr_dev, float beta1, float beta2, float eps, float max_grad_norm,
+                               const double *sumsq, float grad_scale, const uint32_t *skip_flag,
+                               const sf_adam_wt_tab *tab, double *zero_after, void *stream) {
+    SF_REQUIRE(p && g && m && v && P > 0 && step >= 1, "sf_adam_step_wt: bad args");
+    SF_REQUIRE((((uintptr_t)p | (uintptr_t)g | (uintptr_t)m | (uintptr_t)v) & 15) == 0,
+               "sf_adam_step_wt: buffers must be 16-byte aligned");
+    SF_REQUIRE(tab && tab->count >= 0 && tab->count <= SF_ADAM_MAX_WT && (tab->count == 0 || pt),
+               "sf_adam_step_wt: a table of at most %d transposed layers (and their buffer) is required", SF_ADAM_MAX_WT);
+    SF_REQUIRE(!zero_after || zero_after != sumsq, "sf_adam_step_wt: zero_after must not be the slot this step reads");
+    AdamWtPlan t = {};
+    int64_t at = 0;
+    for (int l = 0; l < tab->count; ++l) {
+        const int64_t off = tab->offset[l], KN = (int64_t)tab->K[l] * tab->N[l];
+        SF_REQUIRE(tab->K[l] > 0 && tab->N[l] > 0 && off >= at && off + KN <= P,
+                   "sf_adam_step_wt: layer %d (offset %lld, %d x %d) must lie inside the buffer, in ascending order, "
+                   "without overlap", l, (long long)off, tab->K[l], tab->N[l]);
+        if (off > at) { t.plo[t.nplain] = at; t.phi[t.nplain] = off; ++t.nplain; }
+        t.off[l] = off; t.K[l] = tab->K[l]; t.N[l] = tab->N[l];
+        const int64_t tiles = (int64_t)((tab->K[l] + 31) / 32) * ((tab->N[l] + 31) / 32);
+        SF_REQUIRE(t.tile0[l] + tiles < (1 << 30), "sf_adam_step_wt: too many tiles");
+        t.tile0[l + 1] = t.tile0[l] + (int)tiles;
+        at = off + KN;
+    }
+    if (at < P) { t.plo[t.nplain] = at; t.phi[t.nplain] = P; ++t.nplain; }
+    t.nwt = tab->count;
+    int64_t plain = 0;
+    for (int s = 0; s < t.nplain; ++s) plain += t.phi[s] - t.plo[s];
+    const int64_t pb = (plain / 4 + 255) / 256;
+    const int nplain_blocks = plain == 0 ? 0 : (int)(pb < 2048 ? (pb ? pb : 1) : 2048);
+    AdamC c;
+    const double bc1 = 1.0 - pow((double)beta1, (double)step), bc2 = 1.0 - pow((double)beta2, (double)step);
+    c.lr_step = (float)((double)lr / bc1);
+    c.bc2_sqrt = (float)sqrt(bc2);
+    c.w1 = (float)(1.0 - (double)beta1);
+    c.b2 = beta2;
+    c.w2 = (float)(1.0 - (double)beta2);
+    c.eps = eps;
+    c.max_norm = max_grad_norm;
+    c.grad_scale = grad_scale;
+    k_adam_wt<<<dim3((unsigned)(t.tile0[t.nwt] + nplain_blocks)), dim3(256), 0, STREAM(stream)>>>(
+        p, g, m, v, pt, c, sumsq, skip_flag, lr_dev, t, zero_after);
+    return sf_launch_status("sf_adam_step_wt");
 }
 
 __global__ void k_clock_probe(unsigned long long *__restrict__ out, int spin_cycles) {
diff --git a/sample_factory_amd/lib.py b/sample_factory_amd/lib.py
--- a/sample_factory_amd/lib.py
+++ b/sample_factory_amd/lib.py
@@ -40,7 +40,8 @@
 SYMBOLS = [
     "sf_last_error", "sf_abi_version", "sf_valid_mask", "sf_gae_returns", "sf_moments", "sf_rms_update",
     "sf_rms_apply", "sf_vtrace", "sf_ppo_loss", "sf_loss_scalars", "sf_train_summaries", "sf_minibatch_indices", "sf_minibatch_expand", "sf_grad_sumsq",
-    "sf_adam_step", "sf_adam_step_dlr", "sf_lr_kl_adaptive", "sf_clock_probe", "sf_lamb_step", "sf_rnn_cell_fwd", "sf_rnn_cell_bwd", "sf_rows_add_scale", "sf_mlp2_fwd", "sf_rnn_store_state", "sf_rnn_chunk_setup", "sf_lstm_seq_supported", "sf_lstm_seq_fwd", "sf_lstm_seq_bwd", "sf_gru_seq_fwd", "sf_gru_seq_bwd", "sf_seq_fwd_x_supported", "sf_lstm_seq_fwd_x", "sf_gru_seq_fwd_x", "sf_linear_fwd_dual_supported", "sf_linear_fwd_dual",
+    "sf_adam_step", "sf_adam_step_dlr", "sf_adam_step_wt", "sf_reduce_jobs_create", "sf_reduce_jobs_destroy", "sf_reduce_defer_begin",
+    "sf_reduce_jobs_add", "sf_reduce_partials_batch", "sf_reduce_partials", "sf_moments_acc", "sf_ppo_loss_acc", "sf_loss_scalars_clear", "sf_lr_kl_adaptive", "sf_clock_probe", "sf_lamb_step", "sf_rnn_cell_fwd", "sf_rnn_cell_bwd", "sf_rows_add_scale", "sf_mlp2_fwd", "sf_rnn_store_state", "sf_rnn_chunk_setup", "sf_lstm_seq_supported", "sf_lstm_seq_fwd", "sf_lstm_seq_bwd", "sf_gru_seq_fwd", "sf_gru_seq_bwd", "sf_seq_fwd_x_supported", "sf_lstm_seq_fwd_x", "sf_gru_seq_fwd_x", "sf_linear_fwd_dual_supported", "sf_linear_fwd_dual",
     "sf_obsnorm_moments", "sf_obsnorm_update", "sf_obsnorm_apply", "sf_sample_write_step",
     "sf_sample_write_step_tuple", "sf_sample_write_step_masked", "sf_traj_write_env_step", "sf_synth_obs",
     "sf_synth_step", "sf_synth_vec_step", "sf_h2d_rows", "sf_copy_rows", "sf_conv_fwd", "sf_conv_fwd_workspace", "sf_conv_wgrad_workspace", "sf_conv_wgrad",
@@ -288,9 +289,10 @@
                                  ptr(returns, "f32", "returns"), stream()), "sf_gae_returns")
 
 
-def moments(x, valids, index, n, out, offset=0, dense_x=False) -> None:
-    _check(load().sf_moments(ptr(x, "f32", "x"), ptr(valids, "u8", "valids"), ptr(index, "i32", "index"), i64(offset),
-                             i64(n), int(bool(dense_x)), ptr(out, "f64", "moments"), stream()), "sf_moments")
+def moments(x, valids, index, n, out, offset=0, dense_x=False, acc=False) -> None:
+    fn = load().sf_moments_acc if acc else load().sf_moments
+    _check(fn(ptr(x, "f32", "x"), ptr(valids, "u8", "valids"), ptr(index, "i32", "index"), i64(offset),
+              i64(n), int(bool(dense_x)), ptr(out, "f64", "moments"), stream()), "sf_moments")
 
 
 def rms_update(stats_in, mom, stats_out) -> None:
@@ -497,20 +499,21 @@
 
 
 def ppo_loss(params, ld_params, values, ld_values, actions, old_logp, old_params, old_values, adv, targets, valids,
-             index, offset, n, A, cfg: sf_loss_cfg, mom, sums, g_params, g_values, ratio_out=None) -> None:
-    _check(load().sf_ppo_loss(_raw(params, "f32", "params"), int(ld_params), _raw(values, "f32", "values"),
-                              int(ld_values), ptr(actions, "f32", "actions"), ptr(old_logp, "f32", "old_logp"),
-                              ptr(old_params, "f32", "old_params"), ptr(old_values, "f32", "old_values"),
-                              ptr(adv, "f32", "adv"), ptr(targets, "f32", "targets"), ptr(valids, "u8", "valids"),
-                              ptr(index, "i32", "index"), i64(offset), i64(n), int(A), C.byref(cfg),
-                              ptr(mom, "f64", "moments"), ptr(sums, "f64", "sums"), _raw(g_params, "f32", "g_params"),
-                              _raw(g_values, "f32", "g_values"), ptr(ratio_out, "f32", "ratio_out"), stream()),
+             index, offset, n, A, cfg: sf_loss_cfg, mom, sums, g_params, g_values, ratio_out=None, acc=False) -> None:
+    fn = load().sf_ppo_loss_acc if acc else load().sf_ppo_loss
+    _check(fn(_raw(params, "f32", "params"), int(ld_params), _raw(values, "f32", "values"),
+              int(ld_values), ptr(actions, "f32", "actions"), ptr(old_logp, "f32", "old_logp"),
+              ptr(old_params, "f32", "old_params"), ptr(old_values, "f32", "old_values"),
+              ptr(adv, "f32", "adv"), ptr(targets, "f32", "targets"), ptr(valids, "u8", "valids"),
+              ptr(index, "i32", "index"), i64(offset), i64(n), int(A), C.byref(cfg),
+              ptr(mom, "f64", "moments"), ptr(sums, "f64", "sums"), _raw(g_params, "f32", "g_params"),
+              _raw(g_values, "f32", "g_values"), ptr(ratio_out, "f32", "ratio_out"), stream()),
            "sf_ppo_loss")
 
 
-def loss_scalars(sums, mom, cfg: sf_loss_cfg, out) -> None:
-    _check(load().sf_loss_scalars(ptr(sums, "f64"), ptr(mom, "f64"), C.byref(cfg), ptr(out, "f32"), stream()),
-           "sf_loss_scalars")
+def loss_scalars(sums, mom, cfg: sf_loss_cfg, out, clear=False) -> None:
+    fn = load().sf_loss_scalars_clear if clear else load().sf_loss_scalars
+    _check(fn(ptr(sums, "f64"), ptr(mom, "f64"), C.byref(cfg), ptr(out, "f32"), stream()), "sf_loss_scalars")
 
 
 def train_summaries(valids, ratio, values, ld_values, old_values, old_values_T, actions, num_actions, adv, dense_adv,
@@ -542,7 +545,11 @@
            "sf_grad_sumsq")
 
 
-def adam_step(p, g, m, v, step, lr, beta1, beta2, eps, max_grad_norm, sumsq, grad_scale=1.0, skip_flag=None) -> None:
+def adam_step(p, g, m, v, step, lr, beta1, beta2, eps, max_grad_norm, sumsq, grad_scale=1.0, skip_flag=None,
+              pt=None, wt_tab=None, zero_after=None) -> None:
+    if wt_tab is not None:
+        return adam_step_wt(p, g, m, v, pt, step, lr, None, beta1, beta2, eps, max_grad_norm, sumsq, wt_tab,
+                            zero_after=zero_after, grad_scale=grad_scale, skip_flag=skip_flag)
     _check(load().sf_adam_step(ptr(p, "f32", "params"), ptr(g, "f32", "grads"), ptr(m, "f32", "exp_avg"),
                                ptr(v, "f32", "exp_avg_sq"), i64(p.numel()), int(step), f(lr), f(beta1), f(beta2),
                                f(eps), f(max_grad_norm), ptr(sumsq, "f64", "sumsq"), f(grad_scale),
@@ -551,11 +558,71 @@
 
 
 def adam_step_dlr(p, g, m, v, step, lr_dev, lr_scale, beta1, beta2, eps, max_grad_norm, sumsq, grad_scale=1.0,
-                  skip_flag=None) -> None:
+                  skip_flag=None, pt=None, wt_tab=None, zero_after=None) -> None:
+    if wt_tab is not None:
+        return adam_step_wt(p, g, m, v, pt, step, lr_scale, lr_dev, beta1, beta2, eps, max_grad_norm, sumsq, wt_tab,
+                            zero_after=zero_after, grad_scale=grad_scale, skip_flag=skip_flag)
     _check(load().sf_adam_step_dlr(ptr(p, "f32", "params"), ptr(g, "f32", "grads"), ptr(m, "f32", "exp_avg"),
                                    ptr(v, "f32", "exp_avg_sq"), i64(p.numel()), int(step), ptr(lr_dev, "f32", "lr_dev"),
                                    f(lr_scale), f(beta1), f(beta2), f(eps), f(max_grad_norm), ptr(sumsq, "f64", "sumsq"),
                                    f(grad_scale), ptr(skip_flag, "i32", "skip_flag"), stream()), "sf_adam_step_dlr")
+
+
+ADAM_MAX_WT = 8
+
+
+class sf_adam_wt_tab(C.Structure):
+    _fields_ = [("count", C.c_int32), ("K", C.c_int32 * ADAM_MAX_WT), ("N", C.c_int32 * ADAM_MAX_WT),
+                ("reserved_", C.c_int32), ("offset", C.c_int64 * ADAM_MAX_WT)]
+
+
+def adam_step_wt(p, g, m, v, pt, step, lr, lr_dev, beta1, beta2, eps, max_grad_norm, sumsq, tab: sf_adam_wt_tab,
+                 zero_after=None, grad_scale=1.0, skip_flag=None) -> None:
+    _check(load().sf_adam_step_wt(ptr(p, "f32", "params"), ptr(g, "f32", "grads"), ptr(m, "f32", "exp_avg"),
+                                  ptr(v, "f32", "exp_avg_sq"), ptr(pt, "f32", "params_t"), i64(p.numel()), int(step),
+                                  f(lr), ptr(lr_dev, "f32", "lr_dev"), f(beta1), f(beta2), f(eps), f(max_grad_norm),
+                                  ptr(sumsq, "f64", "sumsq"), f(grad_scale), ptr(skip_flag, "i32", "skip_flag"),
+                                  C.byref(tab), ptr(zero_after, "f64", "zero_after"), stream()), "sf_adam_step_wt")
+
+
+class ReduceJobs:
+
+    def __init__(self):
+        self.h = C.c_void_p()
+        _check(load().sf_reduce_jobs_create(C.byref(self.h)), "sf_reduce_jobs_create")
+
+    def begin(self, sumsq=None) -> None:
+        self._sumsq = sumsq
+        _check(load().sf_reduce_defer_begin(self.h, ptr(sumsq, "f64", "sumsq")), "sf_reduce_defer_begin")
+
+    def add(self, partial, out, n, Z) -> None:
+        _check(load().sf_reduce_jobs_add(self.h, ptr(partial, "f32", "partial"), ptr(out, "f32", "out"), i64(n), int(Z),
+                                         stream()), "sf_reduce_jobs_add")
+
+    def run(self, grads=None) -> None:
+        _check(load().sf_reduce_partials_batch(self.h, ptr(grads, "f32", "grads"),
+                                               i64(grads.numel() if grads is not None else 0), stream()),
+               "sf_reduce_partials_batch")
+
+    def __del__(self):
+        h, self.h = getattr(self, "h", None), None
+        if h and _lib is not None:
+            _lib.sf_reduce_jobs_destroy(h)
+
+
+def reduce_partials(partial, out, n, Z) -> None:
+    _check(load().sf_reduce_partials(ptr(partial, "f32", "partial"), ptr(out, "f32", "out"), i64(n), int(Z), stream()),
+           "sf_reduce_partials")
+
+
+def fuse_tail() -> int:
+    global _FUSE_TAIL
+    if _FUSE_TAIL is None:
+        _FUSE_TAIL = int(os.environ.get("SF_FUSE_TAIL", "15"), 0)
+    return _FUSE_TAIL
+
+
+_FUSE_TAIL: Optional[int] = None
 
 
 def lr_kl_adaptive(kl, lr_dev, threshold, lr_min, lr_max, lr_out=None) -> None:
diff --git a/sample_factory_amd/model/actor_critic.py b/sample_factory_amd/model/actor_critic.py
--- a/sample_factory_amd/model/actor_critic.py
+++ b/sample_factory_amd/model/actor_critic.py
@@ -130,6 +130,8 @@
         return t
 
     def _workspace(self, nbytes: int) -> torch.Tensor:
+        if getattr(self._tls, "defer", None) is not None:
+            return self._defer_slice(nbytes)
         key = getattr(self._tls, "role", "learner")
         ws = self._wss.get(key)
         if ws is None or ws.numel() < nbytes:
@@ -137,6 +139,48 @@
             self._wss[key] = ws
             self._layout_gen += 1
         return ws
+
+    def defer_reductions(self, jobs, sumsq=None) -> None:
+        self._tls.defer, self._tls.defer_off = jobs, 0
+        self._tls.defer_chunk = 0
+        jobs.begin(sumsq)
+
+    def run_reductions(self, with_norm: bool) -> None:
+        jobs, self._tls.defer = self._tls.defer, None
+        jobs.run(self.flat_grads if with_norm else None)
+        if self.nonadaptive_std:
+            assert not with_norm, "the norm is taken after the log-stddev columns are cleared"
+            self._zero_logstd_grads()
+        chunks = self._wss.get("defer")
+        if chunks is not None and len(chunks) > 1:
+            self._wss["defer"] = [torch.empty(sum(c.numel() for c in chunks), dtype=torch.uint8, device=self.device)]
+            self._layout_gen += 1
+
+    def _zero_logstd_grads(self) -> None:
+        A = self.num_action_params
+        self.layers[-1].gw[:, 1 + A // 2:1 + A].zero_()
+
+    def _defer_slice(self, nbytes: int) -> torch.Tensor:
+        nbytes = (max(int(nbytes), 16) + 255) // 256 * 256
+        chunks = self._wss.setdefault("defer", [])
+        ci, off = self._tls.defer_chunk, self._tls.defer_off
+        while ci < len(chunks) and off + nbytes > chunks[ci].numel():
+            ci, off = ci + 1, 0
+        if ci == len(chunks):
+            chunks.append(torch.empty(nbytes, dtype=torch.uint8, device=self.device))
+            self._layout_gen += 1
+        self._tls.defer_chunk, self._tls.defer_off = ci, off + nbytes
+        return chunks[ci][off:off + nbytes]
+
+    def adam_wt_table(self):
+        rows = sorted((o, L.K, L.N) for L, (o, _) in zip(self.layers, self._segs) if L.wt is not None)
+        if len(rows) > lib.ADAM_MAX_WT:
+            return None
+        tab = lib.sf_adam_wt_tab()
+        tab.count = len(rows)
+        for i, (o, K, N) in enumerate(rows):
+            tab.offset[i], tab.K[i], tab.N[i] = o, K, N
+        return tab
 
     def launch_key(self, tag: str = "inf"):
         return (self._layout_gen, self.snap_read if self._snap is not None else -1)
@@ -831,8 +875,7 @@
                     g = gs
                 if pos == 0:
                     self.g_input = g
-            if self.nonadaptive_std and li == len(self.layers) - 1:
-                A = self.num_action_params
-                L.gw[:, 1 + A // 2:1 + A].zero_()
+            if self.nonadaptive_std and li == len(self.layers) - 1 and getattr(self._tls, "defer", None) is None:
+                self._zero_logstd_grads()
             if on_layer_done is not None:
                 on_layer_done(li)
```

After: 2.098 million. About the same (-0.4%).
